# lucasjinreal/yolov7_d2

Hardware: AMD Instinct MI355X
Metric: images/sec training, YOLOX-s 640x640 bs=16/GPU (higher is better)
Workload: dtype bf16; 1 GPU; YOLOX-s CSPDarknet+PAFPN 640x640 bs=16/GPU: fwd + SimOTA loss + bwd + grad all-reduce + SGD(momentum) step, uint8 image batch + labels resident in HBM; global_batch=16, parallelism=dp1, hipgraph=True

## Files before the change

include/mi355_det.h:

```cpp
#ifndef MI355_DET_H
#define MI355_DET_H

#include <stdint.h>

#ifdef __cplusplus
extern "C" {
#endif

#define MI_OK 0
#define MI_EINVAL (-1)
#define MI_ELAUNCH (-2)
#define MI_ENODEV (-3)

typedef void* mi_stream_t;

int mi_version(void);
int mi_device_count(void);
const char* mi_last_error(void);

#define MI_CONV_ACCUM 1
#define MI_CONV_OUT_F32 2
#define MI_CONV_RELU 8
#define MI_CONV_RELUMASK 16
#define MI_CONV_ADDRELU 32
// ... 23 lines not shown
  int32_t KC, BN;
  int32_t stats_slots;
  int32_t TPS;
  const void* bn_y;
  const float* bn_scale;
  const float* bn_shift;
  const float* bn_mean;
  const float* bn_invstd;
  int32_t bn_ldy, bn_act;
  const void* xf;
  int32_t xf_write, xf_C;
} mi_conv_desc;

typedef struct mi_bnx {
  const void* res_unused; void* a;
  const float* gamma; const float* beta; float* rmean; float* rvar; int64_t* nbt;
  float* scale; float* shift; float* mean; float* invstd;
  int32_t ldres_unused, lda, act, pad0_;
  double inv_count, unbias;
  float eps, momentum;
  const double* acc;
  int32_t sld, nslots, C, pad1_;
} mi_bnx;

int mi_conv2d(const mi_conv_desc* d, mi_stream_t s);
int mi_conv2d_plan(mi_conv_desc* d);
int mi_conv2d_route(const mi_conv_desc* d);

#define MI_CONV_MAX_GROUP 8
typedef struct mi_conv_group {
  int32_t njobs, nblocks, lds_bytes;
  int32_t KC, BN, TPIX, TPS, EPI;
  int64_t starts_off, table_bytes;
  int64_t priv[288];
} mi_conv_group;
int mi_conv2d_group_plan(const mi_conv_desc* descs, int n, void* table_host, int64_t table_cap, mi_conv_group* meta);
int mi_conv2d_group_run(const mi_conv_group* meta, const void* table_dev, mi_stream_t s);

struct mi_bn_job;
int mi_conv2d_bn_plan(const mi_conv_desc* descs, const struct mi_bn_job* bn, int n, mi_conv_group* meta);
int mi_conv2d_bn_fwd(const mi_conv_desc* descs, const struct mi_bn_job* bn, int n, mi_stream_t s);
int mi_conv_bn_barrier_status(uint32_t* flags);

int mi_conv1x1_stream(const mi_conv_desc* descs, int n, mi_stream_t s);

int mi_conv3x3_ws(const mi_conv_desc* descs, int n, mi_stream_t s);

typedef struct mi_wgrad_desc {
  const void* x;
  const void* dy;
  float* gw;
  void* ws;
  int64_t ws_bytes;
  int32_t ldx, ldy;
  int32_t N, H, W, outH, outW;
  int32_t stride;
  int32_t Cin, Cout;
  int32_t CinPad, CoutPad;
  int32_t ntaps;
  int32_t tap_dy[MI_MAX_TAPS], tap_dx[MI_MAX_TAPS];
  int32_t accumulate;
  int32_t TH, TW, splitk, cfg_tp, cfg_ns;
  const float* row_scale;
  float* gbias;
} mi_wgrad_desc;
int mi_conv2d_wgrad(const mi_wgrad_desc* d, mi_stream_t s);
int64_t mi_conv2d_wgrad_plan(const mi_wgrad_desc* d);

#define MI_WGRAD_MAX_GROUPS 32
typedef struct mi_wgrad_group {
  int32_t ngroups, nred, red_blocks, pad_;
  struct {
    int32_t cfg[6];
    int32_t njobs, nblocks, lds_bytes, fixup;
    int64_t job_off, starts_off;
  } g[MI_WGRAD_MAX_GROUPS];
  int64_t red_off, red_starts_off, table_bytes, ws_bytes;
  int64_t red9_off, red9_starts_off;
  int32_t nred9, red9_blocks;
} mi_wgrad_group;
int mi_conv2d_wgrad_group_plan(const mi_wgrad_desc* descs, int n, void* ws_base, void* table_host,
                               int64_t table_cap, mi_wgrad_group* meta);
int mi_conv2d_wgrad_group_run(const mi_wgrad_group* meta, const void* table_dev, mi_stream_t s);
int mi_upload_async(void* dst_dev, const void* src_pinned, int64_t nbytes, mi_stream_t s);

int mi_pack_conv_weight(const float* w_oihw, int Cout, int Cin, int KH, int KW,
                        void* wf, int CinPad, int CoutPad,
                        void* wd, int CoutPadK, int CinPadN, mi_stream_t s);

int mi_pack_conv_weight_scaled(const float* w_oihw, const float* cout_scale, int Cout, int Cin, int KH, int KW,
                               void* wf, int CinPad, int CoutPad,
                               void* wd, int CoutPadK, int CinPadN, mi_stream_t s);
int mi_scale_rows_f32(const float* g, const float* scale, float* out, int rows, int rowlen, mi_stream_t s);

typedef struct mi_pack_job {
  const float* w;
  void* wf;
  void* wd;
  int32_t Cout, Cin, KK, CinPad, CoutPad, CoutPadK, CinPadN;
  int32_t blk0;
  const float* scale;
} mi_pack_job;
int mi_pack_jobs_layout(mi_pack_job* jobs_host, int njobs);
int mi_pack_conv_weights_batch(const mi_pack_job* jobs_dev, int njobs, int total_blocks, int kk_max, mi_stream_t s);

int mi_dwconv3x3_fwd(const void* x, int ldx, const float* w, void* y, int ldy, int N, int H, int W, int C, int stride,
                     int outH, int outW, double* stats_acc, int nslots, mi_stream_t s);
int mi_dwconv3x3_dgrad(const void* dy, int lddy, const float* w, void* dx, int lddx, int N, int H, int W, int C,
                       int stride, int outH, int outW, int accumulate, mi_stream_t s);
int64_t mi_dwconv3x3_wgrad_ws_bytes(int C);
int mi_dwconv3x3_wgrad(const void* x, int ldx, const void* dy, int lddy, int N, int H, int W, int C, int stride,
                       int outH, int outW, float* ws, int64_t ws_bytes, float* dw, mi_stream_t s);

#define MI_BN_MAX_GROUP 8
typedef struct mi_bn_job {
  const void* y; const void* res; void* a;
  const void* da; void* dy; void* dres;
  double* acc;
  const float* gamma; const float* beta; float* rmean; float* rvar; int64_t* nbt;
  float* scale; float* shift; float* mean; float* invstd; float* dgamma; float* dbeta;
  int64_t npix, count;
  int32_t ldy, ldres, lda, ldda, lddy, lddres, dres_accum, C, nslots, nblk, act, pad_;
  float eps, momentum;
  uint32_t* bar;
} mi_bn_job;
typedef struct mi_bn_group {
  int32_t kind, njobs, nblocks, act;
  int64_t starts_off, table_bytes;
} mi_bn_group;
int mi_bn_group_plan(int kind, const mi_bn_job* jobs, int n, void* table_host, int64_t table_cap, mi_bn_group* meta);
int mi_bn_group_run(const mi_bn_group* meta, const void* table_dev, mi_stream_t s);

int mi_bn_eval_affine(const float* gamma, const float* beta, const float* running_mean,
                      const float* running_var, float eps, int C, float* scale, float* shift,
                      mi_stream_t s);
int mi_bn_act_fwd(const void* y, int ldy, const double* stats_acc, int nslots, int64_t count, const float* gamma,
                  const float* beta, float eps, float momentum, float* running_mean, float* running_var,
                  int64_t* num_batches_tracked, float* scale, float* shift, float* mean, float* invstd,
                  const void* res, int ldres, void* a, int lda, int64_t npix, int C, int act, mi_stream_t s);
int mi_bn_act_bwd_reduce(const void* da, int ldda, const void* y, int ldy, const float* scale,
                         const float* shift, const float* mean, const float* invstd,
                         double* dacc, int nslots, int nblk, int64_t npix, int C, int act, mi_stream_t s);
int mi_bn_act_bwd_apply(const void* da, int ldda, const void* y, int ldy, const float* scale,
                        const float* shift, const float* mean, const float* invstd,
                        const float* gamma, const double* dacc, int nslots, int64_t count, float* dgamma,
                        float* dbeta,
                        void* dy, int lddy, void* dres, int lddres, int dres_accum, int64_t npix, int C, int act,
                        mi_stream_t s);
#define MI_BN_BAR_GROUPS 16
#define MI_BN_BAR_WORDS (64 * (1 + 2 * MI_BN_BAR_GROUPS))
int mi_bn_fused_set_capacity(int blocks);
int mi_bn_act_bwd_fused(const void* da, int ldda, const void* y, int ldy, const float* scale, const float* shift,
                        const float* mean, const float* invstd, const float* gamma, double* dacc, int nslots,
                        int64_t count, float* dgamma, float* dbeta, void* dy, int lddy, void* dres, int lddres,
                        int dres_accum, int64_t npix, int C, int act, uint32_t* barrier_words, mi_stream_t s);

int mi_focus_pack(const float* img_nchw, int N, int H, int W, void* out, int ldo, mi_stream_t s);
int mi_focus_pack_u8(const uint8_t* img_nchw, int N, int H, int W, void* out, int ldo, mi_stream_t s);
int mi_upsample2x_fwd(const void* x, int ldx, void* y, int ldy, int N, int H, int W, int C,
                      mi_stream_t s);
int mi_upsample2x_bwd(const void* dy, int lddy, void* dx, int lddx, int accumulate, int N, int H,
                      int W, int C, mi_stream_t s);
int mi_spp_pool_fwd(const void* x, int ldx, void* y5, void* y9, void* y13, int ldy, uint8_t* idx,
                    int N, int H, int W, int C, mi_stream_t s);
int mi_spp_pool_bwd(const void* dy5, const void* dy9, const void* dy13, int lddy,
                    const uint8_t* idx, void* dx, int lddx, int accumulate, int N, int H, int W,
// ... 161 lines not shown
} mi_mixup_job;
int mi_mixup_jobs_layout(mi_mixup_job* jobs_host, int njobs);
int mi_mixup_blend(const mi_mixup_job* jobs_dev, int njobs, int total_blocks, mi_stream_t s);

typedef struct mi_pil_resize_job {
  const void* src;
  void* tmp;
  void* dst;
  int64_t dsc, dsy, dsx;
  int64_t src_ld;
  double sat_src;
  int32_t h0, w0, nh, nw;
  int32_t hflip, vflip, shift_x, shift_y;
  int32_t src_hflip;
  int32_t color;
  float sat_dst, bri_dst;
  float dis_hue, dis_sat, dis_exp;
  int32_t dis_pos;
  int32_t blk0h, blk0v;
} mi_pil_resize_job;
int mi_pil_resize_jobs_layout(mi_pil_resize_job* jobs_host, int njobs, int32_t* blocks_h, int32_t* blocks_v);
int mi_pil_resize_h(const mi_pil_resize_job* jobs_dev, int njobs, int total_blocks, mi_stream_t s);
int mi_pil_resize_v(const mi_pil_resize_job* jobs_dev, int njobs, int total_blocks, mi_stream_t s);

typedef struct mi_jpeg_info {
  int32_t width, height, ncomp, restart_interval, orientation, adobe_transform;
  int32_t progressive, pad0_;
  int32_t comp_id[3], hs[3], vs[3], tq[3];
  int32_t hmax, vmax, mcu_w, mcu_h;
  int32_t blocks_w[3], blocks_h[3];
  int64_t coef_off[3], coef_count, sos_pos;
  uint16_t qt[4][64];
  uint8_t dc_bits[4][17], dc_vals[4][256], ac_bits[4][17], ac_vals[4][256];
  uint8_t have_qt[4], have_dc[4], have_ac[4], pad_[4];
} mi_jpeg_info;
typedef struct mi_jpeg_job {
  const int16_t* coef;
  void* planes;
  void* out;
  int64_t coef_off[3], plane_off[3];
  int32_t width, height, ncomp, orientation, bgr, ycc;
  int32_t hs[3], vs[3], blocks_w[3], blocks_h[3];
  int32_t hmax, vmax;
  int32_t blk0_idct, blk0_pix;
  uint16_t qt[3][64];
} mi_jpeg_job;
int mi_jpeg_parse(const uint8_t* data, int64_t len, mi_jpeg_info* info);
int mi_jpeg_huffman(const uint8_t* data, int64_t len, const mi_jpeg_info* info, int16_t* coef_host);
int mi_jpeg_huffman_batch(const uint8_t* const* datas, const int64_t* lens, const mi_jpeg_info* infos, int16_t* const* coefs_host,
                          int n, int threads, int32_t* rcs);
int mi_jpeg_job_fill(const mi_jpeg_info* info, const void* coef_dev, void* planes_dev, void* out_dev, int bgr,
                     int apply_orientation, mi_jpeg_job* job);
int mi_jpeg_jobs_layout(mi_jpeg_job* jobs_host, int njobs, int32_t* blocks_idct, int32_t* blocks_pix);
int mi_jpeg_idct(const mi_jpeg_job* jobs_dev, int njobs, int total_blocks, mi_stream_t s);
int mi_jpeg_color(const mi_jpeg_job* jobs_dev, int njobs, int total_blocks, mi_stream_t s);

int mi_rle_encode(const uint8_t* masks, int n, int H, int W, int max_runs, uint32_t* counts, int32_t* nruns, mi_stream_t s);
int mi_rle_to_string(const uint32_t* counts, int nruns, char* out, int out_cap);

int mi_batched_nms(const float* boxes, const float* scores, const float* idxs, int n, float iou_thr,
                   int32_t* order, uint64_t* mask, float* sboxes, int64_t* keep, int32_t* n_keep,
                   mi_stream_t s);
int mi_batched_nms_ex(const float* boxes, const float* scores, const float* idxs, int n, float iou_thr, int arithmetic,
                      int32_t* order, uint64_t* mask, float* sboxes, int64_t* keep, int32_t* n_keep, mi_stream_t s);
int64_t mi_yolox_postprocess_ws_bytes(int B, int A, int C);
int mi_yolox_postprocess(float* pred, int B, int A, int C, int ld, float conf_thr, float nms_thr, float* dets,
                         int32_t* counts, void* ws, int64_t ws_bytes, mi_stream_t s);
int mi_batched_softnms(const float* boxes, float* scores, const float* idxs, int n, float sigma, float score_threshold,
                       int linear, int64_t* keep, int32_t* n_keep, mi_stream_t s);
int mi_mask_nms(const float* inter, const float* sum_masks, const float* labels, int n, float nms_thr, uint8_t* keep,
                mi_stream_t s);
int mi_matrix_nms(const float* inter, const float* sum_masks, const float* labels, const float* scores, int n, float sigma,
                  int linear, float* comp_ws, float* out_scores, mi_stream_t s);

typedef struct mi_sgd_seg {
  int64_t offset, count;
  float weight_decay, lr;
} mi_sgd_seg;
int mi_sgd_momentum_step(float* params, const float* grads, float* momentum_buf,
                         const mi_sgd_seg* segs_dev, int nseg, float momentum, float grad_scale,
                         int first_step, mi_stream_t s);

int mi_sigmoid_f32(const float* x, const float* dy, float* y, float* dx, int64_t n, mi_stream_t s);
int mi_adamw_step(float* params, const float* grads, float* exp_avg, float* exp_avg_sq, const mi_sgd_seg* segs_dev,
                  int nseg, float beta1, float beta2, float eps, int64_t step, float grad_scale, mi_stream_t s);
typedef struct mi_adamw_tensor {
  float* p; const float* g; float* m; float* v;
  int64_t count;
  float lr, weight_decay;
} mi_adamw_tensor;
typedef struct mi_adamw_chunk {
  int32_t tensor, count;
  int64_t offset;
} mi_adamw_chunk;
int mi_adamw_step_multi(const mi_adamw_tensor* tensors_dev, const mi_adamw_chunk* chunks_dev, int nchunks, float beta1,
                        float beta2, float eps, const int64_t* step_dev, float grad_scale, mi_stream_t s);
int mi_grad_norm_multi(const mi_adamw_tensor* tensors_dev, const mi_adamw_chunk* chunks_dev, int nchunks,
                       double* partial_dev, float max_norm, float grad_scale, float* coef_norm_out, mi_stream_t s);
int mi_grad_gather_multi(const mi_adamw_tensor* tensors_dev, const mi_adamw_chunk* chunks_dev, int nchunks,
                         const int64_t* flat_off_dev, float* flat, mi_stream_t s);
int mi_adamw_step_multi_clip(const mi_adamw_tensor* tensors_dev, const mi_adamw_chunk* chunks_dev, int nchunks, float beta1,
                             float beta2, float eps, const int64_t* step_dev, float grad_scale,
                             const float* grad_scale_dev, mi_stream_t s);
int mi_grad_clip_full_model(float* grads, int64_t n, float max_norm, double* ws, float* norm_out, mi_stream_t s);
int mi_pos_embed_sine(const uint8_t* mask, int B, int H, int W, int num_pos_feats, float temperature, int normalize,
                      float scale, int centered, float* out, mi_stream_t s);

int mi_bilinear_resize_bf16(const void* x, int ldx, int N, int H, int W, int C, void* y, int ldy, int Ho, int Wo,
                            mi_stream_t s);
int mi_bilinear_resize_bwd_bf16(const void* dy, int lddy, int N, int H, int W, int C, void* dx, int lddx, int Ho, int Wo,
                                float* acc_ws_zeroed, mi_stream_t s);
#define MI_PYR_MAX_STAGES 8
int mi_pyramid_pool_fwd(const void* x, int ldx, int N, int H, int W, int C, int ns, const int* kh, const int* kw, void* const* y,
                        mi_stream_t s);
int mi_pyramid_pool_bwd(void* const* dy, int N, int H, int W, int C, int ns, const int* kh, const int* kw, void* dx, int lddx,
                        mi_stream_t s);
int64_t mi_sparseinst_mask_stats_ws_floats(int K, int P);
int mi_sparseinst_mask_stats(const void* masks, int ldm, int P, const float* targets, const int32_t* pairs, int K,
                             float* stats, float* ws, mi_stream_t s);
int mi_sparseinst_mask_grad(const void* masks, int ldm, int P, const float* targets, const int32_t* pairs, int K,
                            const float* stats, float c_bce, float c_dice, void* dmasks_zeroed, mi_stream_t s);
int mi_sparseinst_mask_grad_dev(const void* masks, int ldm, int P, const float* targets, const int32_t* pairs, int K,
                                const float* stats, const float* coef_dev, void* dmasks, mi_stream_t s);

typedef struct mi_sparseinst_loss_desc {
  const float* logits;
  const float* scores;
  const int64_t* labels;
  const int64_t* match_q;
  const int64_t* match_t;
  const int32_t* nmatch;
  const float* inv_num;
  const float* stats;
  const float* gup;
  int32_t* pairs;
  float* valid;
  int32_t* row_cls;
  int32_t* row_pair;
  float* kdev;
  float* losses;
  float* dlogits;
  float* dscores;
  float* coef;
  int B, N, C, cap, P, use_labels, use_masks, pad_;
  float alpha, gamma, w_ce, w_mask, w_dice, w_obj;
} mi_sparseinst_loss_desc;
int mi_sparseinst_match_cost(const float* num, const float* s2, const float* t2, const float* logits, const int64_t* labels,
                             int B, int N, int Np, int C, int cap, float alpha, float beta, float* cost, mi_stream_t s);
int mi_sparseinst_pairs(const mi_sparseinst_loss_desc* d, mi_stream_t s);
int mi_sparseinst_head_loss(const mi_sparseinst_loss_desc* d, mi_stream_t s);
int mi_sparseinst_head_loss_bwd(const mi_sparseinst_loss_desc* d, mi_stream_t s);

int mi_box_convert(const float* in, float* out, int64_t n, int to_cxcywh, mi_stream_t s);
int mi_box_iou_pairwise(const float* boxes1, int n, const float* boxes2, int m, float* iou, float* uni, float* giou,
                        int32_t* degenerate, mi_stream_t s);

int mi_abi_sizeof(int which);

typedef struct mi_cmd {
  int32_t op;
  int32_t i[40];
  float f[8];
  void* p[16];
  int64_t l[4];
} mi_cmd;

enum {
  MI_OP_NOP = 0,
  MI_OP_CONV = 1,
  MI_OP_WGRAD = 2,
  MI_OP_PACK_W = 3,
  MI_OP_RESERVED4 = 4,
  MI_OP_RESERVED5 = 5,
  MI_OP_BN_ACT_FWD = 6,
  MI_OP_BN_BWD_REDUCE = 7,
  MI_OP_RESERVED8 = 8,
  MI_OP_BN_BWD_APPLY = 9,
  MI_OP_FOCUS = 10,
  MI_OP_UPSAMPLE_FWD = 11,
  MI_OP_UPSAMPLE_BWD = 12,
  MI_OP_SPP_FWD = 13,
  MI_OP_SPP_BWD = 14,
  MI_OP_COPY = 15,
  MI_OP_COLSUM = 16,
  MI_OP_LOSS_FWD = 17,
  MI_OP_LOSS_BWD = 18,
  MI_OP_SPLIT_DPREDS = 19,
  MI_OP_MEMSET = 20,
  MI_OP_SGD = 21,
  MI_OP_BN_EVAL_AFFINE = 22,
  MI_OP_DECODE = 23,
  MI_OP_PACK_W_BATCH = 24,
  MI_OP_WGRAD_GROUP = 25,
  MI_OP_RESERVED26 = 26,
  MI_OP_RESERVED27 = 27,
  MI_OP_RESERVED28 = 28,
  MI_OP_BIAS_GRADS = 29,
  MI_OP_CONV_GROUP = 30,
  MI_OP_BN_GROUP = 31,
  MI_OP_SPLIT_DPREDS_BATCH = 32,
  MI_OP_BN_BWD_FUSED = 33,
  MI_OP_DWCONV_FWD = 34,
  MI_OP_DWCONV_DGRAD = 35,
  MI_OP_DWCONV_WGRAD = 36,
  MI_OP_LOSS_BWD_FUSED = 37,
  MI_OP_COUNT
};

int mi_cmdlist_run(const mi_cmd* cmds, int n, mi_stream_t s);
int64_t mi_graph_capture(const mi_cmd* cmds, int n, mi_stream_t s);
int mi_graph_launch(int64_t handle, mi_stream_t s);
int mi_graph_destroy(int64_t handle);

int mi_cmdlist_time(const mi_cmd* cmds, int n, int iters, float* ms, float* per_cmd_ms, mi_stream_t s);

#define MI_FEED_MAX_IMAGES 32
#define MI_FEED_MAX_LEVELS 8
typedef struct mi_image_job {
  const void* src;
  int h, w, dtype, pad_;
} mi_image_job;
typedef struct mi_mask_job {
  const void* masks;
  const int64_t* labels;
  int M, h, w, dtype;
} mi_mask_job;
int mi_normalize_pad_batch(const mi_image_job* jobs, int B, float* dst, int Hp, int Wp, const float* mean3, const float* std3,
                           mi_stream_t s);
int mi_padding_masks(const int64_t* sizes_dev, int B, int nlev, void* const* out, const int* H, const int* W, const int* stride,
                     mi_stream_t s);
int mi_mask_targets_batch(const mi_mask_job* jobs, int B, int cap, int Hi, int Wi, int Ho, int Wo, float* tgt, void* tgtT_bf16,
                          int64_t* labels, float* t2, float* t2_ws, mi_stream_t s);

#define MI_POLY_MAX_H 3807
typedef struct mi_poly_job {
  const double* verts;
  const int32_t* ring_off;
  const int32_t* inst_off;
  const int32_t* ring_off_host;
  const int32_t* inst_off_host;
  void* out;
  int M, h, w, pad_;
} mi_poly_job;
int mi_polygon_masks(const mi_poly_job* jobs, int B, mi_stream_t s);

typedef struct mi_sparseinst_infer_desc {
  int64_t out_off;
  int32_t n, h_img, w_img, Hout, Wout, pad_;
} mi_sparseinst_infer_desc;
int64_t mi_sparseinst_infer_ws_bytes(int B, int N, int h, int w);
int mi_sparseinst_infer_select(const float* logits, const float* obj, const void* masks, int mask_dtype, int64_t sb, int64_t sq,
                               int64_t sy, int64_t sx, int B, int N, int C, int h, int w, float cls_thr, float mask_thr,
                               int* counts, int* kept_query, float* scores, int64_t* labels, void* ws, int64_t ws_bytes,
                               mi_stream_t s);
int mi_sparseinst_infer_masks(const void* masks, int mask_dtype, int64_t sb, int64_t sq, int64_t sy, int64_t sx, int B, int N,
                              int h, int w, int Hpad, int Wpad, const int* kept_query, const mi_sparseinst_infer_desc* descs,
                              float mask_thr, void* out, int64_t out_bytes, mi_stream_t s);

int mi_probe_mfma32(const void* a_bf16_32x16, const void* b_bf16_16x32, float* d_32x32, mi_stream_t s);
int mi_probe_mfma16(const void* a_bf16_16x32, const void* b_bf16_32x16, float* d_16x16, mi_stream_t s);

#ifdef __cplusplus
}
#endif
#endif
```

yolov7_d2_amd/_lib.py:

```python
import ctypes as C
import os

_HERE = os.path.dirname(os.path.abspath(__file__))
LIB_PATH = os.environ.get("MI355_LIB", os.path.join(_HERE, "libmi355det.so"))

MI_MAX_TAPS = 16
MI_CONV_ACCUM = 1
MI_CONV_RELU = 8
MI_CONV_RELUMASK = 16
MI_CONV_ADDRELU = 32
MI_CONV_BNBWD = 4
MI_CONV_OUT_F32 = 2
MI_BN_BAR_WORDS = 64 * (1 + 2 * 16)
MI_BN_SLOTS = 16


class MI355Error(RuntimeError):
    pass


class mi_conv_desc(C.Structure):
    _fields_ = [
        ("x", C.c_void_p), ("w", C.c_void_p), ("y", C.c_void_p), ("bias", C.c_void_p),
        ("stats_acc", C.c_void_p),
# ... 44 lines not shown
                ("lr", C.c_float), ("weight_decay", C.c_float)]


class mi_adamw_chunk(C.Structure):
    _fields_ = [("tensor", C.c_int32), ("count", C.c_int32), ("offset", C.c_int64)]


class mi_bn_job(C.Structure):
    _fields_ = [(n, C.c_void_p) for n in ("y", "res", "a", "da", "dy", "dres", "acc", "gamma", "beta", "rmean", "rvar",
                                          "nbt", "scale", "shift", "mean", "invstd", "dgamma", "dbeta")] + \
               [("npix", C.c_int64), ("count", C.c_int64)] + \
               [(n, C.c_int32) for n in ("ldy", "ldres", "lda", "ldda", "lddy", "lddres", "dres_accum", "C", "nslots",
                                         "nblk", "act", "pad_")] + [("eps", C.c_float), ("momentum", C.c_float), ("bar", C.c_void_p)]


class mi_bn_group(C.Structure):
    _fields_ = [("kind", C.c_int32), ("njobs", C.c_int32), ("nblocks", C.c_int32), ("act", C.c_int32),
                ("starts_off", C.c_int64), ("table_bytes", C.c_int64)]


class mi_wgrad_desc(C.Structure):
    _fields_ = [
        ("x", C.c_void_p), ("dy", C.c_void_p), ("gw", C.c_void_p), ("ws", C.c_void_p), ("ws_bytes", C.c_int64),
        ("ldx", C.c_int32), ("ldy", C.c_int32),
        ("N", C.c_int32), ("H", C.c_int32), ("W", C.c_int32), ("outH", C.c_int32), ("outW", C.c_int32),
        ("stride", C.c_int32), ("Cin", C.c_int32), ("Cout", C.c_int32), ("CinPad", C.c_int32), ("CoutPad", C.c_int32),
        ("ntaps", C.c_int32),
        ("tap_dy", C.c_int32 * MI_MAX_TAPS), ("tap_dx", C.c_int32 * MI_MAX_TAPS),
        ("accumulate", C.c_int32),
        ("TH", C.c_int32), ("TW", C.c_int32), ("splitk", C.c_int32), ("cfg_tp", C.c_int32), ("cfg_ns", C.c_int32),
        ("row_scale", C.c_void_p), ("gbias", C.c_void_p),
    ]


class mi_yolox_loss_desc(C.Structure):
    _fields_ = [
        ("preds", C.c_void_p), ("labels", C.c_void_p), ("anchors", C.c_void_p),
        ("B", C.c_int32), ("A", C.c_int32), ("ncls", C.c_int32), ("max_labels", C.c_int32),
        ("gmax", C.c_int32),
        ("cost", C.c_void_p), ("iou", C.c_void_p), ("match", C.c_void_p), ("ngt", C.c_void_p),
        ("fg", C.c_void_p), ("matched_gt", C.c_void_p), ("matched_iou", C.c_void_p),
        ("partial", C.c_void_p), ("out", C.c_void_p), ("use_l1", C.c_int32), ("rsv_", C.c_int32), ("partial_l1", C.c_void_p),
        ("center_radius", C.c_float), ("cls_weight", C.c_float), ("iou_weight", C.c_float), ("reg_weight", C.c_float),
        ("iou_type", C.c_int32), ("rsv2_", C.c_int32),
    ]


class mi_sgd_seg(C.Structure):
    _fields_ = [("offset", C.c_int64), ("count", C.c_int64), ("weight_decay", C.c_float), ("lr", C.c_float)]


MI_WGRAD_MAX_GROUPS = 32


class _mi_wgrad_group_g(C.Structure):
    _fields_ = [("cfg", C.c_int32 * 6), ("njobs", C.c_int32), ("nblocks", C.c_int32), ("lds_bytes", C.c_int32),
                ("fixup", C.c_int32), ("job_off", C.c_int64), ("starts_off", C.c_int64)]


class mi_wgrad_group(C.Structure):
    _fields_ = [("ngroups", C.c_int32), ("nred", C.c_int32), ("red_blocks", C.c_int32), ("pad_", C.c_int32),
                ("g", _mi_wgrad_group_g * MI_WGRAD_MAX_GROUPS),
                ("red_off", C.c_int64), ("red_starts_off", C.c_int64), ("table_bytes", C.c_int64),
                ("ws_bytes", C.c_int64), ("red9_off", C.c_int64), ("red9_starts_off", C.c_int64),
                ("nred9", C.c_int32), ("red9_blocks", C.c_int32)]


class mi_bias_job(C.Structure):
    _fields_ = [("out", C.c_void_p), ("a0", C.c_int32), ("HW", C.c_int32), ("c0", C.c_int32), ("nc", C.c_int32)]


class mi_split_job(C.Structure):
    _fields_ = [("dst", C.c_void_p), ("a0", C.c_int32), ("HW", C.c_int32), ("c0", C.c_int32), ("nc", C.c_int32),
                ("ld", C.c_int32), ("rsv_", C.c_int32)]


class mi_pack_job(C.Structure):
    _fields_ = [("w", C.c_void_p), ("wf", C.c_void_p), ("wd", C.c_void_p),
                ("Cout", C.c_int32), ("Cin", C.c_int32), ("KK", C.c_int32), ("CinPad", C.c_int32),
                ("CoutPad", C.c_int32), ("CoutPadK", C.c_int32), ("CinPadN", C.c_int32), ("blk0", C.c_int32),
                ("scale", C.c_void_p)]


class mi_sparseinst_loss_desc(C.Structure):
    _fields_ = [(n, C.c_void_p) for n in ("logits", "scores", "labels", "match_q", "match_t", "nmatch", "inv_num", "stats", "gup",
                                          "pairs", "valid", "row_cls", "row_pair", "kdev", "losses", "dlogits", "dscores", "coef")] + \
               [(n, C.c_int32) for n in ("B", "N", "C", "cap", "P", "use_labels", "use_masks", "pad_")] + \
               [(n, C.c_float) for n in ("alpha", "gamma", "w_ce", "w_mask", "w_dice", "w_obj")]


class mi_image_job(C.Structure):
    _fields_ = [("src", C.c_void_p), ("h", C.c_int32), ("w", C.c_int32), ("dtype", C.c_int32), ("pad_", C.c_int32)]


class mi_mask_job(C.Structure):
    _fields_ = [("masks", C.c_void_p), ("labels", C.c_void_p), ("M", C.c_int32), ("h", C.c_int32), ("w", C.c_int32), ("dtype", C.c_int32)]


class mi_poly_job(C.Structure):
    _fields_ = [("verts", C.c_void_p), ("ring_off", C.c_void_p), ("inst_off", C.c_void_p), ("ring_off_host", C.c_void_p),
                ("inst_off_host", C.c_void_p), ("out", C.c_void_p), ("M", C.c_int32), ("h", C.c_int32), ("w", C.c_int32), ("pad_", C.c_int32)]


class mi_sparseinst_infer_desc(C.Structure):
    _fields_ = [("out_off", C.c_int64)] + [(n, C.c_int32) for n in ("n", "h_img", "w_img", "Hout", "Wout", "pad_")]


class mi_mosaic_paste_job(C.Structure):
    _fields_ = [("src", C.c_void_p), ("canvas", C.c_void_p)] + [(n, C.c_int32) for n in
                ("h0", "w0", "rh", "rw", "cw", "x1a", "y1a", "x2a", "y2a", "x1b", "y1b", "blk0", "fsrc", "pad_")]


class mi_warp_job(C.Structure):
    _fields_ = [("canvas", C.c_void_p), ("out", C.c_void_p), ("minv", C.c_double * 6)] + [(n, C.c_int32) for n in
                ("ch", "cw", "h", "w", "Hp", "Wp", "border", "blk0")]


class mi_mixup_job(C.Structure):
    _fields_ = [("src", C.c_void_p), ("out", C.c_void_p)] + [(n, C.c_int32) for n in
                ("h0", "w0", "rh1", "rw1", "dh", "dw", "oh", "ow", "flip", "x_off", "y_off", "th", "tw", "Hp", "Wp", "blk0", "fsrc", "pad_")]


class mi_pil_resize_job(C.Structure):
    _fields_ = ([("src", C.c_void_p), ("tmp", C.c_void_p), ("dst", C.c_void_p), ("dsc", C.c_int64), ("dsy", C.c_int64),
                 ("dsx", C.c_int64), ("src_ld", C.c_int64), ("sat_src", C.c_double)] +
                [(n, C.c_int32) for n in ("h0", "w0", "nh", "nw", "hflip", "vflip", "shift_x", "shift_y", "src_hflip", "color")] +
                [("sat_dst", C.c_float), ("bri_dst", C.c_float), ("dis_hue", C.c_float), ("dis_sat", C.c_float), ("dis_exp", C.c_float),
                 ("dis_pos", C.c_int32), ("blk0h", C.c_int32), ("blk0v", C.c_int32)])


class mi_jpeg_info(C.Structure):
    _fields_ = ([(n, C.c_int32) for n in ("width", "height", "ncomp", "restart_interval", "orientation", "adobe_transform",
                                         "progressive", "pad0_")] +
                [(n, C.c_int32 * 3) for n in ("comp_id", "hs", "vs", "tq")] +
                [(n, C.c_int32) for n in ("hmax", "vmax", "mcu_w", "mcu_h")] +
                [("blocks_w", C.c_int32 * 3), ("blocks_h", C.c_int32 * 3), ("coef_off", C.c_int64 * 3), ("coef_count", C.c_int64),
                 ("sos_pos", C.c_int64), ("qt", (C.c_uint16 * 64) * 4), ("dc_bits", (C.c_uint8 * 17) * 4),
                 ("dc_vals", (C.c_uint8 * 256) * 4), ("ac_bits", (C.c_uint8 * 17) * 4), ("ac_vals", (C.c_uint8 * 256) * 4),
                 ("have_qt", C.c_uint8 * 4), ("have_dc", C.c_uint8 * 4), ("have_ac", C.c_uint8 * 4), ("pad_", C.c_uint8 * 4)])


class mi_jpeg_job(C.Structure):
    _fields_ = ([("coef", C.c_void_p), ("planes", C.c_void_p), ("out", C.c_void_p), ("coef_off", C.c_int64 * 3),
                 ("plane_off", C.c_int64 * 3)] +
                [(n, C.c_int32) for n in ("width", "height", "ncomp", "orientation", "bgr", "ycc")] +
                [(n, C.c_int32 * 3) for n in ("hs", "vs", "blocks_w", "blocks_h")] +
                [(n, C.c_int32) for n in ("hmax", "vmax", "blk0_idct", "blk0_pix")] + [("qt", (C.c_uint16 * 64) * 3)])


class mi_cmd(C.Structure):
    _fields_ = [("op", C.c_int32), ("i", C.c_int32 * 40), ("f", C.c_float * 8), ("p", C.c_void_p * 16),
                ("l", C.c_int64 * 4)]


OPS = ["NOP", "CONV", "WGRAD", "PACK_W", "RESERVED4", "RESERVED5", "BN_ACT_FWD", "BN_BWD_REDUCE",
       "RESERVED8", "BN_BWD_APPLY", "FOCUS", "UPSAMPLE_FWD", "UPSAMPLE_BWD", "SPP_FWD", "SPP_BWD", "COPY",
       "COLSUM", "LOSS_FWD", "LOSS_BWD", "SPLIT_DPREDS", "MEMSET", "SGD", "BN_EVAL_AFFINE", "DECODE", "PACK_W_BATCH", "WGRAD_GROUP", "RESERVED26", "RESERVED27", "RESERVED28", "BIAS_GRADS",
       "CONV_GROUP", "BN_GROUP", "SPLIT_DPREDS_BATCH", "BN_BWD_FUSED", "DWCONV_FWD", "DWCONV_DGRAD", "DWCONV_WGRAD",
       "LOSS_BWD_FUSED"]
OP = {n: k for k, n in enumerate(OPS)}

_vp, _i, _i64, _f = C.c_void_p, C.c_int, C.c_int64, C.c_float
_PROTOS = {
    "mi_version": (C.c_int, []),
    "mi_device_count": (C.c_int, []),
    "mi_last_error": (C.c_char_p, []),
    "mi_conv2d": (C.c_int, [C.POINTER(mi_conv_desc), _vp]),
    "mi_conv2d_plan": (C.c_int, [C.POINTER(mi_conv_desc)]),
    "mi_conv2d_wgrad": (C.c_int, [C.POINTER(mi_wgrad_desc), _vp]),
    "mi_conv2d_wgrad_group_plan": (C.c_int, [C.POINTER(mi_wgrad_desc), _i, _vp, _vp, _i64, C.POINTER(mi_wgrad_group)]),
    "mi_conv2d_wgrad_group_run": (C.c_int, [C.POINTER(mi_wgrad_group), _vp, _vp]),
    "mi_pack_conv_weight": (C.c_int, [_vp, _i, _i, _i, _i, _vp, _i, _i, _vp, _i, _i, _vp]),
    "mi_pack_conv_weight_scaled": (C.c_int, [_vp, _vp, _i, _i, _i, _i, _vp, _i, _i, _vp, _i, _i, _vp]),
    "mi_scale_rows_f32": (C.c_int, [_vp, _vp, _vp, _i, _i, _vp]),
    "mi_conv2d_wgrad_plan": (C.c_int64, [C.POINTER(mi_wgrad_desc)]),
    "mi_bn_eval_affine": (C.c_int, [_vp, _vp, _vp, _vp, _f, _i, _vp, _vp, _vp]),
    "mi_bn_act_fwd": (C.c_int, [_vp, _i, _vp, _i, _i64, _vp, _vp, _f, _f, _vp, _vp, _vp, _vp, _vp, _vp, _vp, _vp, _i, _vp, _i,
                                _i64, _i, _i, _vp]),
    "mi_bn_act_bwd_reduce": (C.c_int, [_vp, _i, _vp, _i, _vp, _vp, _vp, _vp, _vp, _i, _i, _i64, _i, _i, _vp]),
    "mi_bn_act_bwd_apply": (C.c_int, [_vp, _i, _vp, _i, _vp, _vp, _vp, _vp, _vp, _vp, _i, _i64, _vp, _vp, _vp, _i, _vp, _i, _i,
                                      _i64, _i, _i, _vp]),
    "mi_focus_pack": (C.c_int, [_vp, _i, _i, _i, _vp, _i, _vp]),
    "mi_focus_pack_u8": (C.c_int, [_vp, _i, _i, _i, _vp, _i, _vp]),
    "mi_maxpool3x3s2_fwd": (C.c_int, [_vp, _i, _vp, _i, _i, _i, _i, _i, _vp]),
    "mi_maxpool3x3s2_bwd": (C.c_int, [_vp, _i, _vp, _i, _vp, _i, _i, _i, _i, _i, _i, _vp]),
    "mi_maxpool3x3s2_fwd_idx": (C.c_int, [_vp, _i, _vp, _i, _vp, _i, _i, _i, _i, _vp]),
    "mi_maxpool3x3s2_bwd_idx": (C.c_int, [_vp, _vp, _i, _vp, _i, _i, _i, _i, _i, _i, _vp]),
    "mi_upsample2x_fwd": (C.c_int, [_vp, _i, _vp, _i, _i, _i, _i, _i, _vp]),
    "mi_upsample2x_bwd": (C.c_int, [_vp, _i, _vp, _i, _i, _i, _i, _i, _i, _vp]),
    "mi_spp_pool_fwd": (C.c_int, [_vp, _i, _vp, _vp, _vp, _i, _vp, _i, _i, _i, _i, _vp]),
    "mi_spp_pool_bwd": (C.c_int, [_vp, _vp, _vp, _i, _vp, _vp, _i, _i, _i, _i, _i, _i, _vp]),
    "mi_copy_bf16": (C.c_int, [_vp, _i, _vp, _i, _i, _i64, _i, _vp]),
    "mi_colsum_bf16": (C.c_int, [_vp, _i, _i64, _i, _vp, _i, _vp, _vp]),
    "mi_colsum_bf16_wide": (C.c_int, [_vp, _i, _i64, _i, _vp, _i, _vp, _vp]),
    "mi_colsumsq_bf16_wide": (C.c_int, [_vp, _i, _i64, _i, _vp, _i, _vp, _vp]),
    "mi_colsum_wide_ws_bytes": (C.c_int64, [_i]),
    "mi_pack_conv_weights_batch": (C.c_int, [_vp, _i, _i, _i, _vp]),
    "mi_pack_jobs_layout": (C.c_int, [C.POINTER(mi_pack_job), _i]),
    "mi_yolox_loss_fwd": (C.c_int, [C.POINTER(mi_yolox_loss_desc), _vp]),
    "mi_yolox_loss_bwd": (C.c_int, [C.POINTER(mi_yolox_loss_desc), _vp, _vp, _vp]),
    "mi_yolox_loss_bwd_fused": (C.c_int, [C.POINTER(mi_yolox_loss_desc), _vp, _vp, C.POINTER(mi_split_job), _i,
                                          C.POINTER(mi_bias_job), _i, _vp, _i64, _vp]),
    "mi_yolox_split_dpreds": (C.c_int, [_vp, _i, _i, _i, _i, _i, _i, _i, _vp, _i, _vp]),
    "mi_yolox_split_dpreds_batch": (C.c_int, [_vp, _i, _i, _i, C.POINTER(mi_split_job), _i, _vp]),
    "mi_yolox_bias_grads": (C.c_int, [_vp, _i, _i, _i, C.POINTER(mi_bias_job), _i, _vp, _vp]),
    "mi_yolox_decode": (C.c_int, [_vp, _vp, _i, _i, _i, _vp]),
    "mi_hungarian_match": (C.c_int, [_vp, _vp, _vp, _vp, _vp, _i, _i, _i, _i, _f, _f, _f, _vp, _vp, _vp, _vp, _vp]),
    "mi_lsap": (C.c_int, [_vp, _vp, _i, _i, _i, _vp, _vp, _vp, _vp]),
    "mi_conv2d_group_plan": (C.c_int, [C.POINTER(mi_conv_desc), _i, _vp, _i64, C.POINTER(mi_conv_group)]),
    "mi_conv2d_group_run": (C.c_int, [C.POINTER(mi_conv_group), _vp, _vp]),
    "mi_conv2d_route": (C.c_int, [C.POINTER(mi_conv_desc)]),
    "mi_dropout_seed_offset": (C.c_int, [_vp]),
    "mi_adamw_step_multi": (C.c_int, [_vp, _vp, _i, _f, _f, _f, _vp, _f, _vp]),
    "mi_adamw_step_multi_clip": (C.c_int, [_vp, _vp, _i, _f, _f, _f, _vp, _f, _vp, _vp]),
    "mi_grad_norm_multi": (C.c_int, [_vp, _vp, _i, _vp, _f, _f, _vp, _vp]),
    "mi_grad_gather_multi": (C.c_int, [_vp, _vp, _i, _vp, _vp, _vp]),
    "mi_conv2d_bn_plan": (C.c_int, [C.POINTER(mi_conv_desc), C.POINTER(mi_bn_job), _i, C.POINTER(mi_conv_group)]),
    "mi_conv2d_bn_fwd": (C.c_int, [C.POINTER(mi_conv_desc), C.POINTER(mi_bn_job), _i, _vp]),
    "mi_conv_bn_barrier_status": (C.c_int, [C.POINTER(C.c_uint32)]),
    "mi_conv1x1_stream": (C.c_int, [C.POINTER(mi_conv_desc), _i, _vp]),
    "mi_conv3x3_ws": (C.c_int, [C.POINTER(mi_conv_desc), _i, _vp]),
    "mi_bn_act_bwd_fused": (C.c_int, [_vp, _i, _vp, _i, _vp, _vp, _vp, _vp, _vp, _vp, _i, _i64, _vp, _vp, _vp, _i, _vp, _i,
                                      _i, _i64, _i, _i, _vp, _vp]),
    "mi_bn_fused_set_capacity": (C.c_int, [_i]),
    "mi_dwconv3x3_fwd": (C.c_int, [_vp, _i, _vp, _vp, _i, _i, _i, _i, _i, _i, _i, _i, _vp, _i, _vp]),
    "mi_dwconv3x3_dgrad": (C.c_int, [_vp, _i, _vp, _vp, _i, _i, _i, _i, _i, _i, _i, _i, _i, _vp]),
    "mi_dwconv3x3_wgrad_ws_bytes": (C.c_int64, [_i]),
    "mi_dwconv3x3_wgrad": (C.c_int, [_vp, _i, _vp, _i, _i, _i, _i, _i, _i, _i, _i, _vp, _i64, _vp, _vp]),
    "mi_batched_nms_ex": (C.c_int, [_vp, _vp, _vp, _i, _f, _i, _vp, _vp, _vp, _vp, _vp, _vp]),
    "mi_batched_softnms": (C.c_int, [_vp, _vp, _vp, _i, _f, _f, _i, _vp, _vp, _vp]),
    "mi_mask_nms": (C.c_int, [_vp, _vp, _vp, _i, _f, _vp, _vp]),
    "mi_matrix_nms": (C.c_int, [_vp, _vp, _vp, _vp, _i, _f, _i, _vp, _vp, _vp]),
    "mi_groupnorm_ws_bytes": (C.c_int64, [_i, _i]),
    "mi_groupnorm_fwd": (C.c_int, [_vp, _i, _i, _i, _i, _i, _vp, _vp, _f, _vp, _i, _vp, _vp, _vp]),
    "mi_groupnorm_bwd": (C.c_int, [_vp, _i, _vp, _i, _i, _i, _i, _i, _vp, _vp, _vp, _i, _vp, _vp, _vp, _vp]),
    "mi_maxpool2x2_fwd": (C.c_int, [_vp, _i, _vp, _i, _i, _i, _i, _i, _vp]),
    "mi_maxpool2x2_bwd": (C.c_int, [_vp, _i, _vp, _i, _vp, _i, _i, _i, _i, _i, _vp]),
    "mi_fastattn_ws_bytes": (C.c_int64, []),
    "mi_fastattn_fwd": (C.c_int, [C.POINTER(C.c_void_p), _i, _vp, _vp, _i64, _vp]),
    "mi_fastattn_bwd": (C.c_int, [C.POINTER(C.c_void_p), _i, _vp, _vp, C.POINTER(C.c_void_p), _vp, _vp, _i64, _vp]),
    "mi_mosaic_jobs_layout": (C.c_int, [C.POINTER(mi_mosaic_paste_job), _i, C.POINTER(mi_warp_job), _i]),
    "mi_mosaic_paste": (C.c_int, [_vp, _i, _i, _vp]),
    "mi_warp_affine_u8": (C.c_int, [_vp, _i, _i, _vp]),
    "mi_mixup_jobs_layout": (C.c_int, [C.POINTER(mi_mixup_job), _i]),
    "mi_mixup_blend": (C.c_int, [_vp, _i, _i, _vp]),
    "mi_pil_resize_jobs_layout": (C.c_int, [C.POINTER(mi_pil_resize_job), _i, C.POINTER(C.c_int32), C.POINTER(C.c_int32)]),
    "mi_pil_resize_h": (C.c_int, [_vp, _i, _i, _vp]),
    "mi_pil_resize_v": (C.c_int, [_vp, _i, _i, _vp]),
    "mi_jpeg_parse": (C.c_int, [_vp, C.c_int64, C.POINTER(mi_jpeg_info)]),
    "mi_jpeg_huffman": (C.c_int, [_vp, C.c_int64, C.POINTER(mi_jpeg_info), _vp]),
    "mi_jpeg_huffman_batch": (C.c_int, [_vp, _vp, _vp, _vp, _i, _i, _vp]),
    "mi_jpeg_job_fill": (C.c_int, [C.POINTER(mi_jpeg_info), _vp, _vp, _vp, _i, _i, C.POINTER(mi_jpeg_job)]),
    "mi_jpeg_jobs_layout": (C.c_int, [C.POINTER(mi_jpeg_job), _i, C.POINTER(C.c_int32), C.POINTER(C.c_int32)]),
    "mi_jpeg_idct": (C.c_int, [_vp, _i, _i, _vp]),
# ... 130 lines not shown
```

yolov7_d2_amd/csrc/conv_wgrad.hip:

```cpp
#include <stdlib.h>
#include <string.h>
#include <vector>
#include "common.h"

struct Wg2K {
  const __bf16* x;
  const __bf16* dy;
  float* part;
  int ldx, lddy, N, H, W, outH, outW, is;
  int TH, TW, tilesY, tilesX, ntiles, tps, nsplit;
  int dymin, dxmin, haloW, npixh, nqx, stage, ns;
  int toff[MI_MAX_TAPS];
  int nco, nci;
  int nrx;
  int xmap;
  unsigned mTW, mHW;
  long long V;
  float* bpart;
  int bld, fix;
  float* g;
  const float* row_scale;
  int Cout, Cin, accumulate, pad_;
  int ra, rb;
  long long cnt_rel;
};

__device__ uint4 g_mi_zero_page[4];

typedef __attribute__((address_space(3))) s16x4* lds_s16x4_ptr;

__device__ __forceinline__ bf16x8 tr_read2(const char* base0, const char* base1) {
  const s16x4 lo = __builtin_amdgcn_ds_read_tr16_b64_v4i16((lds_s16x4_ptr)(base0));
  const s16x4 hi = __builtin_amdgcn_ds_read_tr16_b64_v4i16((lds_s16x4_ptr)(base1));
  typedef __attribute__((ext_vector_type(8))) short s16x8;
  s16x8 v;
  v[0] = lo[0]; v[1] = lo[1]; v[2] = lo[2]; v[3] = lo[3];
  v[4] = hi[0]; v[5] = hi[1]; v[6] = hi[2]; v[7] = hi[3];
  return __builtin_bit_cast(bf16x8, v);
}

__device__ __forceinline__ void glds16(const void* g, unsigned lds_off) {
  asm volatile("s_mov_b32 m0, %1\n\ts_nop 0\n\tglobal_load_lds_dwordx4 %0, off" ::"v"(g), "s"(__builtin_amdgcn_readfirstlane(lds_off)) : "memory", "m0");
}

__device__ __forceinline__ void wait_vmcnt(int n) {
#define MI_VMC(k) case k: asm volatile("s_waitcnt vmcnt(" #k ")" ::: "memory"); break;
  switch (n < 0 ? 0 : (n > 30 ? 30 : n)) {
    MI_VMC(0) MI_VMC(1) MI_VMC(2) MI_VMC(3) MI_VMC(4) MI_VMC(5) MI_VMC(6) MI_VMC(7) MI_VMC(8) MI_VMC(9) MI_VMC(10)
    MI_VMC(11) MI_VMC(12) MI_VMC(13) MI_VMC(14) MI_VMC(15) MI_VMC(16) MI_VMC(17) MI_VMC(18) MI_VMC(19) MI_VMC(20)
    MI_VMC(21) MI_VMC(22) MI_VMC(23) MI_VMC(24) MI_VMC(25) MI_VMC(26) MI_VMC(27) MI_VMC(28) MI_VMC(29) MI_VMC(30)
  }
#undef MI_VMC
}

template <int NG>
__device__ __forceinline__ int swz32(int row) {
  if (NG == 1) return 0;
  if (NG == 2) return (row >> 2) & 1;
  if (NG == 4) return (row >> 1) & 3;
  return row & 7;
}

template <int NTHR, int BCO>
struct WgBias {
  static constexpr int NCH = BCO / 8, RL = NTHR / NCH;
  float s[8];
  __device__ __forceinline__ void init() {
#pragma unroll
    for (int e = 0; e < 8; ++e) s[e] = 0.f;
  }
  template <int TP>
  __device__ __forceinline__ void tile(const Wg2K& p, const int img, const int ty0, const int tx0, const int co0, const int TPv) {
    const int tid = threadIdx.x, ch = tid % NCH, rl = tid / NCH;
    if (rl >= RL) return;
    const __bf16* const dyb = p.dy + ((size_t)img * p.outH * p.outW) * (size_t)p.lddy + co0 + ch * 8;
    constexpr int NR = (TP + RL - 1) / RL;
    bf16x8 v[NR];
#pragma unroll
    for (int k = 0; k < NR; ++k) {
      const int row = rl + k * RL;
      const int ty = (int)(((unsigned)row * p.mTW) >> 20);
      const int tx = row - ty * p.TW;
      const int oy = ty0 + ty, ox = tx0 + tx;
      const bool ok = (row < TPv) & (oy < p.outH) & (ox < p.outW);
#pragma unroll
      for (int e = 0; e < 8; ++e) v[k][e] = (__bf16)0.f;
// ... 519 lines not shown
#pragma unroll
    for (int ks = 0; ks < KS; ++ks) {
      bf16x8 a[MI];
#pragma unroll
      for (int i = 0; i < MI; ++i)
        a[i] = tr_read2(aB + (i * TP + ks * 32) * 32, aB + (i * TP + ks * 32 + 16) * 32);
      const char* const b0 = sB + hb[ks][0];
      const char* const b1 = sB + hb[ks][1];
#pragma unroll
      for (int tap = 0; tap < NT; ++tap) {
        bf16x8 b[NJ];
#pragma unroll
        for (int j = 0; j < NJ; ++j)
          b[j] = tr_read2(b0 + toff32[tap] + j * jstride, b1 + toff32[tap] + j * jstride);
#pragma unroll
        for (int i = 0; i < MI; ++i)
#pragma unroll
          for (int j = 0; j < NJ; ++j)
            acc[tap][i][j] = __builtin_amdgcn_mfma_f32_16x16x32_bf16(a[i], b[j], acc[tap][i][j], 0, 0, 0);
      }
    }
  }
  f32x4* out = (f32x4*)p.part + (size_t)s * (size_t)p.V +
               ((size_t)((cob * p.nci + cib) * NW + wave) * (NT * MI * NJ)) * 64 + lane;
  if (FIX) {
    const __amdgpu_buffer_rsrc_t rs = wg_slab_rsrc(p.part);
    const unsigned ob = (unsigned)(((size_t)s * (size_t)p.V + ((size_t)((cob * p.nci + cib) * NW + wave) * (NT * MI * NJ)) * 64 + lane) * 16);
#pragma unroll
    for (int tap = 0; tap < NT; ++tap)
#pragma unroll
      for (int i = 0; i < MI; ++i)
#pragma unroll
        for (int j = 0; j < NJ; ++j) st_agent16(rs, ob, (unsigned)(((tap * MI + i) * NJ + j) * 1024), acc[tap][i][j]);
    wg_fixup<NT, MI, NJ, WCO, WCI>(p, cnt, s, cob * p.nci + cib, smem);
    return;
  }
#pragma unroll
  for (int tap = 0; tap < NT; ++tap)
#pragma unroll
    for (int i = 0; i < MI; ++i)
#pragma unroll
      for (int j = 0; j < NJ; ++j) out[((tap * MI + i) * NJ + j) * 64] = acc[tap][i][j];
  if (p.bpart != nullptr) {
    if (do_bias) bias.finish(p, (float*)smem, s, co0);
  }
}

template <int NT, int MI, int NJ, int WCO, int WCI, int TP>
__global__ __launch_bounds__(WCO* WCI * 64, 2) void wgrad3_kernel(const Wg2K p) {
  wgrad3_body<NT, MI, NJ, WCO, WCI, TP>(p, blockIdx.x);
}
template <int NT, int MI, int NJ, int WCO, int WCI, int TP>
__global__ __launch_bounds__(WCO* WCI * 64, 2) void wgrad3_group_kernel(const Wg2K* __restrict__ jobs,
                                                                         const int* __restrict__ starts, int njobs) {
  const int b = blockIdx.x;
  int j = 0;
  while (j + 1 < njobs && starts[j + 1] <= b) ++j;
  const Wg2K p = jobs[j];
  wgrad3_body<NT, MI, NJ, WCO, WCI, TP>(p, b - starts[j]);
}
template <int TP>
__global__ __launch_bounds__(256, 2) void wgrad3_multi_kernel(const Wg2K* __restrict__ jobs, const int* __restrict__ starts, int njobs) {
  const int b = blockIdx.x;
  int j = 0;
  while (j + 1 < njobs && starts[j + 1] <= b) ++j;
  const Wg2K p = jobs[j];
  const int bid = b - starts[j];
  switch (p.pad_) {
    case 0x41: wgrad3_body<9, 4, 1, 1, 4, TP>(p, bid); break;
    case 0x22: wgrad3_body<9, 2, 1, 2, 2, TP>(p, bid); break;
    default: wgrad3_body<9, 1, 1, 2, 2, TP>(p, bid); break;
  }
}
template <int NT, int MI, int NJ, int WCO, int WCI, int TP>
__global__ __launch_bounds__(WCO* WCI * 64, 2) void wgrad3_group_fix_kernel(const Wg2K* __restrict__ jobs,
                                                                             const int* __restrict__ starts, int njobs) {
  const int b = blockIdx.x;
  int j = 0;
  while (j + 1 < njobs && starts[j + 1] <= b) ++j;
  const Wg2K p = jobs[j];
  wgrad3_body<NT, MI, NJ, WCO, WCI, TP, true>(p, b - starts[j], (unsigned*)((char*)const_cast<Wg2K*>(jobs) + p.cnt_rel));
}

struct Wg2R {
  const f32x4* part;
  float* g;
  long long V;
  int nsplit, NT, MI, NJ, WCO, WCI, nco, nci, Cout, Cin, accumulate;
  const float* row_scale;
  const float* bpart;
  float* gbias;
  int bld, main_blocks;
};
__device__ __forceinline__ void wgrad2_reduce_bias(const Wg2R& p, const long long blk) {
  const int c = (int)(blk - p.main_blocks) * 256 + (int)threadIdx.x;
  if (c >= p.Cout) return;
  float a = 0.f;
  for (int k = 0; k < p.nsplit; ++k) a += p.bpart[(size_t)k * p.bld + c];
  p.gbias[c] = a;
}

template <int SL>
__device__ __forceinline__ void wgrad2_reduce_body(const Wg2R& p, const long long blk) {
  constexpr int OUTS = 256 / SL;
  __shared__ f32x4 red[SL > 1 ? SL - 1 : 1][OUTS];
  const int o = threadIdx.x % OUTS, sl = threadIdx.x / OUTS;
  const long long v = blk * OUTS + o;
  const bool valid = v < p.V;
  f32x4 s0 = {0.f, 0.f, 0.f, 0.f}, s1 = s0, s2 = s0, s3 = s0;
  if (valid) {
    const f32x4* src = p.part + v;
    int k = sl;
    for (; k + 3 * SL < p.nsplit; k += 4 * SL) {
      const f32x4 a = src[(size_t)k * p.V], b = src[(size_t)(k + SL) * p.V], c = src[(size_t)(k + 2 * SL) * p.V],
                  d = src[(size_t)(k + 3 * SL) * p.V];
      s0 += a; s1 += b; s2 += c; s3 += d;
    }
    for (; k < p.nsplit; k += SL) s0 += src[(size_t)k * p.V];
  }
  f32x4 sum = (s0 + s1) + (s2 + s3);
  if (SL > 1) {
    if (sl > 0) red[sl - 1][o] = sum;
    __syncthreads();
    if (sl > 0) return;
#pragma unroll
    for (int q = 0; q < SL - 1; ++q) sum += red[q][o];
  }
  if (!valid) return;
  wg_scatter(p.g, p.row_scale, p.accumulate, p.NT, p.MI, p.NJ, p.WCO, p.WCI, p.nci, p.Cout, p.Cin, v, sum);
}

__device__ __forceinline__ void wgrad2_reduce9_body(const Wg2R& p, const int blk) {
  __shared__ float tile[16 * 16 * 9 + 16];
  const int tid = threadIdx.x, lane = tid & 63, tap = tid >> 6;
  int r = blk;
  const int j = r % p.NJ; r /= p.NJ;
  const int i = r % p.MI; r /= p.MI;
  const int NW = p.WCO * p.WCI;
  const int wave = r % NW; r /= NW;
  const int cib = r % p.nci, cob = r / p.nci;
  const long long v = ((((long long)(r * NW + wave) * 9 + tap) * p.MI + i) * p.NJ + j) * 64 + lane;
  f32x4 s0 = {0.f, 0.f, 0.f, 0.f}, s1 = s0, s2 = s0, s3 = s0;
  const f32x4* src = p.part + v;
  int k = 0;
  for (; k + 4 <= p.nsplit; k += 4) {
    const f32x4 a = src[(size_t)k * p.V], b = src[(size_t)(k + 1) * p.V], c = src[(size_t)(k + 2) * p.V],
                d = src[(size_t)(k + 3) * p.V];
    s0 += a; s1 += b; s2 += c; s3 += d;
  }
  for (; k < p.nsplit; ++k) s0 += src[(size_t)k * p.V];
  const f32x4 sum = (s0 + s1) + (s2 + s3);
#pragma unroll
  for (int e = 0; e < 4; ++e) tile[((4 * (lane >> 4) + e) * 16 + (lane & 15)) * 9 + tap] = sum[e];
  __syncthreads();
  const int wco = wave / p.WCI, wci = wave % p.WCI;
  const int ci0 = cib * (16 * p.NJ * p.WCI) + (wci * p.NJ + j) * 16;
  const int co0 = cob * (16 * p.MI * p.WCO) + (wco * p.MI + i) * 16;
  if (ci0 >= p.Cin) return;
  const int row = tid / 36, c4 = (tid % 36) * 4;
  const int co = co0 + row;
  const int nval = min(16, p.Cin - ci0) * 9;
  if (co >= p.Cout || c4 >= nval) return;
  float* dst = p.g + ((size_t)co * p.Cin + ci0) * 9 + c4;
  const float* t = tile + row * 144 + c4;
  const float rs = p.row_scale ? p.row_scale[co] : 1.f;
  if (c4 + 4 <= nval && ((uintptr_t)dst & 15) == 0) {
    f32x4 o = {t[0] * rs, t[1] * rs, t[2] * rs, t[3] * rs};
    if (p.accumulate) o += *(const f32x4*)dst;
    *(f32x4*)dst = o;
  } else {
    for (int e = 0; e < 4 && c4 + e < nval; ++e) dst[e] = p.accumulate ? dst[e] + t[e] * rs : t[e] * rs;
  }
}
__global__ __launch_bounds__(576) void wgrad2_reduce9_kernel(const Wg2R p) { wgrad2_reduce9_body(p, blockIdx.x); }
__global__ __launch_bounds__(576) void wgrad2_reduce9_group_kernel(const Wg2R* __restrict__ jobs,
                                                                   const int* __restrict__ starts, int njobs) {
// ... 442 lines not shown
        done[j] = 1;
        starts.push_back(blocks);
        ks[j].pad_ = cs[j].NT == 9 ? cs[j].MI * 16 + cs[j].WCO : cs[j].MI * 16 + cs[j].NJ;
        if (fix) {
          ks[j].fix = 1;
          ks[j].cnt_rel = (long long)cnt_off[j] - (long long)job_off;
        }
        jobs.push_back(ks[j]);
        blocks += ks[j].nsplit * ks[j].nco * ks[j].nci;
        if (ldss[j] > lds) lds = ldss[j];
      }
    starts.push_back(blocks);
    if (fix) {
      const size_t need = 16 + (size_t)3 * WG_FIX_U * (cs[i].WCO * cs[i].WCI * 16) * 16;
      if (lds < need) lds = need;
    }
    g.njobs = (int)jobs.size(); g.nblocks = blocks; g.lds_bytes = (int32_t)lds; g.fixup = fix ? 1 : 0;
    g.job_off = put(jobs.data(), jobs.size() * sizeof(Wg2K));
    MI_REQUIRE(g.job_off == job_off, "wgrad_group_plan: table layout");
    g.starts_off = put(starts.data(), starts.size() * sizeof(int));
  }
  std::vector<Wg2R> rj, rj9;
  std::vector<int> rs, rs9;
  int rblocks = 0, rblocks9 = 0;
  for (int i = 0; i < n && !fix; ++i) {
    Wg2R r;
    r.part = (const f32x4*)ks[i].part; r.g = descs[i].gw; r.V = ks[i].V; r.nsplit = ks[i].nsplit;
    r.NT = cs[i].NT; r.MI = cs[i].MI; r.NJ = cs[i].NJ; r.WCO = cs[i].WCO; r.WCI = cs[i].WCI;
    r.nco = ks[i].nco; r.nci = ks[i].nci; r.Cout = descs[i].Cout; r.Cin = descs[i].Cin;
    r.accumulate = descs[i].accumulate; r.row_scale = descs[i].row_scale;
    r.bpart = nullptr; r.gbias = nullptr; r.bld = 0; r.main_blocks = 0;
    if (descs[i].gbias) {
      const int outs = 256 / wg_redsl();
      r.bpart = ks[i].bpart; r.gbias = descs[i].gbias; r.bld = ks[i].bld;
      r.main_blocks = (int)((ks[i].V + outs - 1) / outs);
      rj.push_back(r);
      rs.push_back(rblocks);
      rblocks += r.main_blocks + (descs[i].Cout + 255) / 256;
      continue;
    }
    if (cs[i].NT == 9 && wg_red9()) {
      rj9.push_back(r);
      rs9.push_back(rblocks9);
      rblocks9 += (int)(ks[i].V / (64 * 9));
    } else {
      rj.push_back(r);
      rs.push_back(rblocks);
      const int outs = 256 / wg_redsl();
      rblocks += (int)((ks[i].V + outs - 1) / outs);
    }
  }
  rs.push_back(rblocks);
  rs9.push_back(rblocks9);
  meta->nred = (int)rj.size(); meta->red_blocks = rblocks;
  meta->red_off = put(rj.data(), rj.size() * sizeof(Wg2R));
  meta->red_starts_off = put(rs.data(), rs.size() * sizeof(int));
  meta->nred9 = (int)rj9.size(); meta->red9_blocks = rblocks9;
  meta->red9_off = put(rj9.data(), rj9.size() * sizeof(Wg2R));
  meta->red9_starts_off = put(rs9.data(), rs9.size() * sizeof(int));
  meta->table_bytes = (int64_t)off;
  if (tab) MI_REQUIRE((int64_t)off <= table_cap, "wgrad_group_plan: table needs %zu bytes", off);
  return MI_OK;
}

template <int NT, int MI, int NJ, int WCO, int WCI, int TP>
static int wg_group_launch(const Wg2K* jobs, const int* starts, int njobs, int nblocks, size_t lds, hipStream_t s, bool fix) {
  auto fn = fix ? (wg_use_v3(NT) ? wgrad3_group_fix_kernel<NT, MI, NJ, WCO, WCI, TP> : wgrad2_group_fix_kernel<NT, MI, NJ, WCO, WCI, TP>)
                : (wg_use_v3(NT) ? wgrad3_group_kernel<NT, MI, NJ, WCO, WCI, TP> : wgrad2_group_kernel<NT, MI, NJ, WCO, WCI, TP>);
  static bool attr_done = false;
  if (!attr_done) {
    hipFuncSetAttribute((const void*)wgrad2_group_kernel<NT, MI, NJ, WCO, WCI, TP>, hipFuncAttributeMaxDynamicSharedMemorySize, 160 * 1024);
    hipFuncSetAttribute((const void*)wgrad3_group_kernel<NT, MI, NJ, WCO, WCI, TP>, hipFuncAttributeMaxDynamicSharedMemorySize, 160 * 1024);
    hipFuncSetAttribute((const void*)wgrad2_group_fix_kernel<NT, MI, NJ, WCO, WCI, TP>, hipFuncAttributeMaxDynamicSharedMemorySize, 160 * 1024);
    hipFuncSetAttribute((const void*)wgrad3_group_fix_kernel<NT, MI, NJ, WCO, WCI, TP>, hipFuncAttributeMaxDynamicSharedMemorySize, 160 * 1024);
    attr_done = true;
  }
  if ((size_t)wg_min_lds() > lds && wg_min_lds() <= 160 * 1024) lds = (size_t)wg_min_lds();
  hipLaunchKernelGGL(fn, dim3((unsigned)nblocks), dim3(WCO * WCI * 64), lds, s, jobs, starts, njobs);
  MI_CHECK_LAUNCH("conv_wgrad_group");
  return MI_OK;
}

extern "C" int mi_conv2d_wgrad_group_run(const mi_wgrad_group* meta, const void* table_dev, mi_stream_t st) {
  MI_REQUIRE(meta && table_dev && meta->ngroups > 0, "wgrad_group_run: args");
  hipStream_t s = (hipStream_t)st;
  const char* tab = (const char*)table_dev;
  for (int gi = 0; gi < meta->ngroups; ++gi) {
    const auto& g = meta->g[gi];
    const Wg2K* jobs = (const Wg2K*)(tab + g.job_off);
    const int* starts = (const int*)(tab + g.starts_off);
    int rc = MI_EINVAL;
#define MI_WG(NTv, MIv, NJv, WCOv, WCIv, TPv)                                                                   \
  if (g.cfg[0] == NTv && g.cfg[1] == MIv && g.cfg[2] == NJv && g.cfg[3] == WCOv && g.cfg[4] == WCIv &&          \
      g.cfg[5] == TPv)                                                                                          \
    rc = wg_group_launch<NTv, MIv, NJv, WCOv, WCIv, TPv>(jobs, starts, g.njobs, g.nblocks, (size_t)g.lds_bytes, s, g.fixup == 1);
    MI_WG_ALL
#undef MI_WG
    if (g.cfg[0] == 1 && g.cfg[1] == 0 && g.cfg[2] == 0 && g.fixup != 1) {
      static bool attr_done = false;
      if (!attr_done) {
        hipFuncSetAttribute((const void*)wgrad2_multi_kernel<64>, hipFuncAttributeMaxDynamicSharedMemorySize, 160 * 1024);
        hipFuncSetAttribute((const void*)wgrad2_multi_kernel<128>, hipFuncAttributeMaxDynamicSharedMemorySize, 160 * 1024);
        attr_done = true;
      }
      if (g.cfg[5] == 64)
        hipLaunchKernelGGL(wgrad2_multi_kernel<64>, dim3((unsigned)g.nblocks), dim3(256), (size_t)g.lds_bytes, s, jobs, starts, g.njobs);
      else
        hipLaunchKernelGGL(wgrad2_multi_kernel<128>, dim3((unsigned)g.nblocks), dim3(256), (size_t)g.lds_bytes, s, jobs, starts, g.njobs);
      MI_CHECK_LAUNCH("conv_wgrad_multi");
      rc = MI_OK;
    }
    if (g.cfg[0] == 9 && g.cfg[1] == 0 && g.cfg[2] == 0 && g.fixup != 1) {
      static bool attr_done = false;
      if (!attr_done) {
        hipFuncSetAttribute((const void*)wgrad3_multi_kernel<64>, hipFuncAttributeMaxDynamicSharedMemorySize, 160 * 1024);
        hipFuncSetAttribute((const void*)wgrad3_multi_kernel<128>, hipFuncAttributeMaxDynamicSharedMemorySize, 160 * 1024);
        attr_done = true;
      }
      if (g.cfg[5] == 64)
        hipLaunchKernelGGL(wgrad3_multi_kernel<64>, dim3((unsigned)g.nblocks), dim3(256), (size_t)g.lds_bytes, s, jobs, starts, g.njobs);
      else
        hipLaunchKernelGGL(wgrad3_multi_kernel<128>, dim3((unsigned)g.nblocks), dim3(256), (size_t)g.lds_bytes, s, jobs, starts, g.njobs);
      MI_CHECK_LAUNCH("conv_wgrad3_multi");
      rc = MI_OK;
    }
    if (rc == MI_EINVAL) MI_FAIL(MI_EINVAL, "wgrad_group: no kernel for group %d", gi);
    if (rc) return rc;
  }
  if (meta->red9_blocks > 0) {
    hipLaunchKernelGGL(wgrad2_reduce9_group_kernel, dim3((unsigned)meta->red9_blocks), dim3(576), 0, s,
                       (const Wg2R*)(tab + meta->red9_off), (const int*)(tab + meta->red9_starts_off), meta->nred9);
    MI_CHECK_LAUNCH("conv_wgrad_reduce9_group");
  }
  if (meta->red_blocks > 0) {
    const dim3 g((unsigned)meta->red_blocks);
    const Wg2R* jt = (const Wg2R*)(tab + meta->red_off);
    const int* st_ = (const int*)(tab + meta->red_starts_off);
    switch (wg_redsl()) {
      case 16: hipLaunchKernelGGL(wgrad2_reduce_group_kernel<16>, g, dim3(256), 0, s, jt, st_, meta->nred); break;
      case 8: hipLaunchKernelGGL(wgrad2_reduce_group_kernel<8>, g, dim3(256), 0, s, jt, st_, meta->nred); break;
      case 4: hipLaunchKernelGGL(wgrad2_reduce_group_kernel<4>, g, dim3(256), 0, s, jt, st_, meta->nred); break;
      default: hipLaunchKernelGGL(wgrad2_reduce_group_kernel<1>, g, dim3(256), 0, s, jt, st_, meta->nred);
    }
    MI_CHECK_LAUNCH("conv_wgrad_reduce_group");
  }
  return MI_OK;
}
```

yolov7_d2_amd/csrc/misc_ops.hip:

```cpp
#include <stdlib.h>
#include "common.h"

static int ew_blocks(int64_t total, int cap = 4096) {
  int64_t b = (total + 255) / 256;
  if (b > cap) b = cap;
  if (b < 1) b = 1;
  return (int)b;
}

__global__ __launch_bounds__(256) void focus_pack_kernel(const float* __restrict__ img, int N, int H, int W,
                                                         __bf16* out, int ldo) {
  const int Ho = H / 2, Wo = W / 2;
  const int64_t total = (int64_t)N * Ho * Wo;
  for (int64_t idx = blockIdx.x * 256LL + threadIdx.x; idx < total; idx += (int64_t)gridDim.x * 256) {
    const int ox = (int)(idx % Wo);
    const int64_t r = idx / Wo;
    const int oy = (int)(r % Ho), n = (int)(r / Ho);
    float f[16];
#pragma unroll
    for (int q = 0; q < 4; ++q) {
      const int dy = q & 1, dx = q >> 1;
#pragma unroll
      for (int c = 0; c < 3; ++c)
        f[q * 3 + c] = img[(((int64_t)n * 3 + c) * H + (2 * oy + dy)) * W + 2 * ox + dx];
    }
    f[12] = f[13] = f[14] = f[15] = 0.f;
    __bf16* op = out + idx * ldo;
    *(bf16x8*)op = pack8(f);
    *(bf16x8*)(op + 8) = pack8(f + 8);
  }
}

template <class T>
__global__ __launch_bounds__(256) void focus_pack4_kernel(const T* __restrict__ img, int N, int H, int W, __bf16* out,
                                                          int ldo) {
  const int Ho = H / 2, Wo = W / 2;
  const unsigned total = (unsigned)N * (unsigned)Ho * (unsigned)Wo;
  const unsigned stride = gridDim.x * 256u;
  for (unsigned idx0 = blockIdx.x * 256u + threadIdx.x; idx0 < total; idx0 += 4 * stride) {
    float f[4][16];
#pragma unroll
    for (int j = 0; j < 4; ++j) {
      const unsigned idx = idx0 + j * stride;
      if (idx >= total) break;
      const unsigned r = idx / (unsigned)Wo;
      const int ox = (int)(idx - r * (unsigned)Wo);
      const unsigned nn = r / (unsigned)Ho;
      const int oy = (int)(r - nn * (unsigned)Ho), n = (int)nn;
#pragma unroll
      for (int c = 0; c < 3; ++c)
#pragma unroll
        for (int dy = 0; dy < 2; ++dy) {
          const T* src = img + (((int64_t)n * 3 + c) * H + (2 * oy + dy)) * W + 2 * ox;
          if constexpr (sizeof(T) == 4) {
            const float2 v = *(const float2*)src;
            f[j][dy * 3 + c] = v.x;
            f[j][(2 + dy) * 3 + c] = v.y;
          } else {
            const unsigned short v = *(const unsigned short*)src;
            f[j][dy * 3 + c] = (float)(v & 0xff);
            f[j][(2 + dy) * 3 + c] = (float)(v >> 8);
          }
        }
      f[j][12] = f[j][13] = f[j][14] = f[j][15] = 0.f;
    }
#pragma unroll
    for (int j = 0; j < 4; ++j) {
      const unsigned idx = idx0 + j * stride;
      if (idx >= total) break;
      __bf16* op = out + (size_t)idx * ldo;
      *(bf16x8*)op = pack8(f[j]);
      *(bf16x8*)(op + 8) = pack8(f[j] + 8);
    }
  }
}

#define FOCUS_ROWS 2
__global__ __launch_bounds__(256) void focus_pack_u8_rows_kernel(const uint8_t* __restrict__ img, int N, int H, int W,
                                                                 __bf16* out, int ldo) {
  extern __shared__ __attribute__((aligned(16))) uint8_t srow[];
  const int Ho = H / 2, Wo = W / 2;
  const int rb = (Ho + FOCUS_ROWS - 1) / FOCUS_ROWS;
  const int n = blockIdx.x / rb, oy0 = (blockIdx.x % rb) * FOCUS_ROWS;
  const int per = W / 16;
// ... 700 lines not shown
    const int c = tid & 63, q = tid >> 6, nbk = (int)gridDim.x;
    float a = 0.f;
    if (c < C8N * 8) {
      int b = q;
      for (; b + 12 < nbk; b += 16) {
        float v[4];
#pragma unroll
        for (int u = 0; u < 4; ++u) v[u] = __hip_atomic_load(part + (size_t)(b + 4 * u) * CP + c0 + c, __ATOMIC_RELAXED, __HIP_MEMORY_SCOPE_AGENT);
        a += (v[0] + v[1]) + (v[2] + v[3]);
      }
      for (; b < nbk; b += 4) a += __hip_atomic_load(part + (size_t)b * CP + c0 + c, __ATOMIC_RELAXED, __HIP_MEMORY_SCOPE_AGENT);
    }
    red[q * 64 + c] = a;
    __syncthreads();
    if (tid < C8N * 8 && c0 + tid < C) {
      const float t = (red[tid] + red[64 + tid]) + (red[128 + tid] + red[192 + tid]);
      out[c0 + tid] = accumulate ? out[c0 + tid] + t : t;
    }
  }
}
extern "C" int64_t mi_colsum_wide_ws_bytes(int C) { return (int64_t)128 * ((C + 7) / 8 * 8) * 4; }
static int colsum_wide_launch(const void* x, int ldx, int64_t npix, int C, float* out, int accumulate, float* ws, int sq,
                              mi_stream_t st) {
  MI_REQUIRE(x && out && ws && C > 0, "colsum_wide: null / C %d", C);
  const int CP = (C + 7) / 8 * 8;
  MI_REQUIRE(ldx % 8 == 0 && ((uintptr_t)x % 16) == 0 && ldx >= CP, "colsum_wide: alignment / ld");
  hipStream_t s = (hipStream_t)st;
  int nblk = (int)((npix + 255) / 256);
  if (nblk > 128) nblk = 128;
  if (nblk < 1) nblk = 1;
  const char* two_e = getenv("MI_COLSUM_TWO_STAGE");
  const int two = two_e ? atoi(two_e) : 0;
  if ((CP + 63) / 64 <= COLSUM_MAX_CHUNKS && !two) {
    hipLaunchKernelGGL(colsum_wide_fused_kernel, dim3(nblk, (CP + 63) / 64), dim3(256), 0, s, (const __bf16*)x, ldx, npix, CP, C, ws,
                       out, accumulate, sq);
    MI_CHECK_LAUNCH("colsum_wide");
    return MI_OK;
  }
  hipLaunchKernelGGL(colsum_wide_stage1_kernel, dim3(nblk, (CP + 63) / 64), dim3(256), 0, s, (const __bf16*)x, ldx, npix, CP, ws, sq);
  MI_CHECK_LAUNCH("colsum_wide1");
  hipLaunchKernelGGL(colsum_wide_stage2_kernel, dim3((C + 127) / 128), dim3(128), 0, s, ws, nblk, CP, C, out, accumulate);
  MI_CHECK_LAUNCH("colsum_wide2");
  return MI_OK;
}
extern "C" int mi_colsum_bf16_wide(const void* x, int ldx, int64_t npix, int C, float* out, int accumulate, float* ws,
                                   mi_stream_t st) {
  return colsum_wide_launch(x, ldx, npix, C, out, accumulate, ws, 0, st);
}
extern "C" int mi_colsumsq_bf16_wide(const void* x, int ldx, int64_t npix, int C, float* out, int accumulate, float* ws,
                                     mi_stream_t st) {
  return colsum_wide_launch(x, ldx, npix, C, out, accumulate, ws, 1, st);
}

__global__ __launch_bounds__(256) void scale_rows_kernel(const float* __restrict__ g, const float* __restrict__ sc, float* out,
                                                         int rows, int rowlen) {
  const int64_t n = (int64_t)rows * rowlen;
  if ((rowlen & 3) == 0) {
    const int64_t n4 = n >> 2;
    const int rl4 = rowlen >> 2;
    for (int64_t i = blockIdx.x * 256LL + threadIdx.x; i < n4; i += (int64_t)gridDim.x * 256) {
      const float f = sc[i / rl4];
      float4 v = ((const float4*)g)[i];
      v.x *= f; v.y *= f; v.z *= f; v.w *= f;
      ((float4*)out)[i] = v;
    }
  } else {
    for (int64_t i = blockIdx.x * 256LL + threadIdx.x; i < n; i += (int64_t)gridDim.x * 256) out[i] = g[i] * sc[i / rowlen];
  }
}
extern "C" int mi_scale_rows_f32(const float* g, const float* scale, float* out, int rows, int rowlen, mi_stream_t st) {
  MI_REQUIRE(g && scale && out && rows > 0 && rowlen > 0, "scale_rows: args");
  MI_REQUIRE(((uintptr_t)g % 16) == 0 && ((uintptr_t)out % 16) == 0, "scale_rows: alignment");
  int64_t blocks = ((int64_t)rows * rowlen / 4 + 255) / 256;
  if (blocks > 2048) blocks = 2048;
  if (blocks < 1) blocks = 1;
  hipLaunchKernelGGL(scale_rows_kernel, dim3((int)blocks), dim3(256), 0, (hipStream_t)st, g, scale, out, rows, rowlen);
  MI_CHECK_LAUNCH("scale_rows");
  return MI_OK;
}

__global__ __launch_bounds__(256) void sgd_kernel(float* p, const float* __restrict__ g, float* m,
                                                  const mi_sgd_seg* __restrict__ segs, float momentum,
                                                  float grad_scale, int first_step) {
  const mi_sgd_seg sg = segs[blockIdx.x];
  const float wd = sg.weight_decay, lr = sg.lr;
  const int64_t n4 = ((sg.offset & 3) == 0) ? (sg.count >> 2) : 0;
  f32x4* p4 = (f32x4*)(p + sg.offset);
  const f32x4* g4 = (const f32x4*)(g + sg.offset);
  f32x4* m4 = (f32x4*)(m + sg.offset);
  for (int64_t i = threadIdx.x; i < n4; i += 512) {
    const bool two = i + 256 < n4;
    const f32x4 pa = p4[i], ga = g4[i], ma = first_step ? f32x4{0.f, 0.f, 0.f, 0.f} : m4[i];
    f32x4 pb = {0.f, 0.f, 0.f, 0.f}, gb = pb, mb = pb;
    if (two) {
      pb = p4[i + 256];
      gb = g4[i + 256];
      if (!first_step) mb = m4[i + 256];
    }
    f32x4 da = ga * grad_scale + pa * wd;
    f32x4 ba = first_step ? da : ma * momentum + da;
    m4[i] = ba;
    p4[i] = pa - ba * lr;
    if (two) {
      f32x4 db = gb * grad_scale + pb * wd;
      f32x4 bb = first_step ? db : mb * momentum + db;
      m4[i + 256] = bb;
      p4[i + 256] = pb - bb * lr;
    }
  }
  for (int64_t i = n4 * 4 + threadIdx.x; i < sg.count; i += 256) {
    const int64_t k = sg.offset + i;
    const float pv = p[k];
    const float d = g[k] * grad_scale + wd * pv;
    const float b = first_step ? d : momentum * m[k] + d;
    m[k] = b;
    p[k] = pv - lr * b;
  }
}
extern "C" int mi_sgd_momentum_step(float* params, const float* grads, float* momentum_buf,
                                    const mi_sgd_seg* segs_dev, int nseg, float momentum, float grad_scale,
                                    int first_step, mi_stream_t st) {
  MI_REQUIRE(params && grads && momentum_buf && segs_dev && nseg > 0, "sgd: args");
  hipLaunchKernelGGL(sgd_kernel, dim3(nseg), dim3(256), 0, (hipStream_t)st, params, grads, momentum_buf, segs_dev,
                     momentum, grad_scale, first_step);
  MI_CHECK_LAUNCH("sgd");
  return MI_OK;
}
```

yolov7_d2_amd/csrc/runtime.hip:

```cpp
#include <mutex>
#include <unordered_map>
#include <vector>
#include "common.h"

__global__ __launch_bounds__(256) void fill16_kernel(u32x4* p, size_t n16, unsigned v) {
  const u32x4 w = {v, v, v, v};
  for (size_t k = (size_t)blockIdx.x * 256 + threadIdx.x; k < n16; k += (size_t)gridDim.x * 256) p[k] = w;
}

thread_local char g_mi_err[512] = {0};

extern "C" int mi_version(void) { return 100; }
extern "C" const char* mi_last_error(void) { return g_mi_err; }

const unsigned long long* g_mi_seed_off = nullptr;
extern "C" int mi_dropout_seed_offset(const uint64_t* dev_word) {
  g_mi_seed_off = (const unsigned long long*)dev_word;
  return MI_OK;
}
extern "C" int mi_device_count(void) {
  int n = 0;
  if (hipGetDeviceCount(&n) != hipSuccess) return 0;
  return n;
}

static int run_one(const mi_cmd& c, hipStream_t s) {
  mi_stream_t st = (mi_stream_t)s;
  const int32_t* i = c.i;
  void* const* p = c.p;
  switch (c.op) {
    case MI_OP_NOP: return MI_OK;
    case MI_OP_CONV: return mi_conv2d((const mi_conv_desc*)p[0], st);
    case MI_OP_WGRAD: return mi_conv2d_wgrad((const mi_wgrad_desc*)p[0], st);
    case MI_OP_PACK_W:
      return mi_pack_conv_weight((const float*)p[0], i[0], i[1], i[2], i[3], p[1], i[4], i[5], p[2], i[6], i[7], st);
    case MI_OP_BN_ACT_FWD:
      return mi_bn_act_fwd(p[0], i[0], (const double*)p[1], i[5], c.l[0], (const float*)p[2], (const float*)p[3], c.f[0],
                           c.f[1], (float*)p[4], (float*)p[5], (int64_t*)p[6], (float*)p[7], (float*)p[8],
                           (float*)p[9], (float*)p[10], p[11], i[1], p[12], i[2], c.l[1], i[3], i[4], st);
    case MI_OP_BN_BWD_REDUCE:
      return mi_bn_act_bwd_reduce(p[0], i[0], p[1], i[1], (const float*)p[2], (const float*)p[3], (const float*)p[4],
                                  (const float*)p[5], (double*)p[6], i[5], i[2], c.l[0], i[3], i[4], st);
    case MI_OP_BN_BWD_APPLY:
      return mi_bn_act_bwd_apply(p[0], i[0], p[1], i[1], (const float*)p[2], (const float*)p[3], (const float*)p[4],
                                 (const float*)p[5], (const float*)p[6], (const double*)p[7], i[7], c.l[1], (float*)p[8],
                                 (float*)p[9], p[10], i[2], p[11], i[3], i[4], c.l[0], i[5], i[6], st);
    case MI_OP_BN_BWD_FUSED:
      return mi_bn_act_bwd_fused(p[0], i[0], p[1], i[1], (const float*)p[2], (const float*)p[3], (const float*)p[4],
                                 (const float*)p[5], (const float*)p[6], (double*)p[7], i[7], c.l[1], (float*)p[8],
                                 (float*)p[9], p[10], i[2], p[11], i[3], i[4], c.l[0], i[5], i[6], (uint32_t*)p[12], st);
    case MI_OP_DWCONV_FWD:
      return mi_dwconv3x3_fwd(p[0], i[0], (const float*)p[1], p[2], i[1], i[2], i[3], i[4], i[5], i[6], i[7], i[8],
                              (double*)p[3], i[9], st);
    case MI_OP_DWCONV_DGRAD:
      return mi_dwconv3x3_dgrad(p[0], i[0], (const float*)p[1], p[2], i[1], i[2], i[3], i[4], i[5], i[6], i[7], i[8], i[9], st);
    case MI_OP_DWCONV_WGRAD:
      return mi_dwconv3x3_wgrad(p[0], i[0], p[1], i[1], i[2], i[3], i[4], i[5], i[6], i[7], i[8], (float*)p[2], c.l[0],
                                (float*)p[3], st);
    case MI_OP_FOCUS:
      return i[4] ? mi_focus_pack_u8((const uint8_t*)p[0], i[0], i[1], i[2], p[1], i[3], st)
                  : mi_focus_pack((const float*)p[0], i[0], i[1], i[2], p[1], i[3], st);
    case MI_OP_UPSAMPLE_FWD: return mi_upsample2x_fwd(p[0], i[0], p[1], i[1], i[2], i[3], i[4], i[5], st);
    case MI_OP_UPSAMPLE_BWD: return mi_upsample2x_bwd(p[0], i[0], p[1], i[1], i[2], i[3], i[4], i[5], i[6], st);
    case MI_OP_SPP_FWD: return mi_spp_pool_fwd(p[0], i[0], p[1], p[2], p[3], i[1], (uint8_t*)p[4], i[2], i[3], i[4], i[5], st);
    case MI_OP_SPP_BWD:
      return mi_spp_pool_bwd(p[0], p[1], p[2], i[0], (const uint8_t*)p[3], p[4], i[1], i[2], i[3], i[4], i[5], i[6], st);
    case MI_OP_COPY: return mi_copy_bf16(p[0], i[0], p[1], i[1], i[2], c.l[0], i[3], st);
    case MI_OP_COLSUM: return mi_colsum_bf16(p[0], i[0], c.l[0], i[1], (float*)p[1], i[2], (float*)p[2], st);
    case MI_OP_BIAS_GRADS:
      return mi_yolox_bias_grads((const float*)p[1], i[0], i[1], i[2], (const mi_bias_job*)p[0], i[3], (float*)p[2], st);
    case MI_OP_WGRAD_GROUP: return mi_conv2d_wgrad_group_run((const mi_wgrad_group*)p[0], p[1], st);
    case MI_OP_CONV_GROUP: return mi_conv2d_group_run((const mi_conv_group*)p[0], p[1], st);
    case MI_OP_BN_GROUP: return mi_bn_group_run((const mi_bn_group*)p[0], p[1], st);
    case MI_OP_PACK_W_BATCH: return mi_pack_conv_weights_batch((const mi_pack_job*)p[0], i[0], i[1], i[2], st);
    case MI_OP_LOSS_FWD: return mi_yolox_loss_fwd((const mi_yolox_loss_desc*)p[0], st);
    case MI_OP_LOSS_BWD_FUSED:
      return mi_yolox_loss_bwd_fused((const mi_yolox_loss_desc*)p[0], (const float*)p[1], (float*)p[2], (const mi_split_job*)p[3], i[0],
                                     (const mi_bias_job*)p[4], i[1], (float*)p[5], c.l[0], st);
    case MI_OP_LOSS_BWD: return mi_yolox_loss_bwd((const mi_yolox_loss_desc*)p[0], (const float*)p[1], (float*)p[2], st);
    case MI_OP_SPLIT_DPREDS:
      return mi_yolox_split_dpreds((const float*)p[0], i[0], i[1], i[2], i[3], i[4], i[5], i[6], p[1], i[7], st);
    case MI_OP_SPLIT_DPREDS_BATCH:
      return mi_yolox_split_dpreds_batch((const float*)p[1], i[0], i[1], i[2], (const mi_split_job*)p[0], i[3], st);
    case MI_OP_MEMSET: {
      const size_t n = (size_t)c.l[0];
      if (((uintptr_t)p[0] % 16) == 0 && n % 16 == 0 && n > 0 && n < ((size_t)1 << 40)) {
        const unsigned v = (unsigned)(i[0] & 0xff) * 0x01010101u;
        const size_t n16 = n / 16;
        size_t nb = (n16 + 255) / 256;
        if (nb > 2048) nb = 2048;
        hipLaunchKernelGGL(fill16_kernel, dim3((unsigned)nb), dim3(256), 0, s, (u32x4*)p[0], n16, v);
        MI_CHECK_LAUNCH("memset (fill kernel)");
        return MI_OK;
      }
      if (hipMemsetAsync(p[0], i[0], n, s) != hipSuccess) MI_FAIL(MI_ELAUNCH, "memset failed");
      return MI_OK;
    }
    case MI_OP_SGD:
      return mi_sgd_momentum_step((float*)p[0], (const float*)p[1], (float*)p[2], (const mi_sgd_seg*)p[3], i[0],
                                  c.f[0], c.f[1], i[1], st);
    case MI_OP_BN_EVAL_AFFINE:
      return mi_bn_eval_affine((const float*)p[0], (const float*)p[1], (const float*)p[2], (const float*)p[3], c.f[0],
                               i[0], (float*)p[4], (float*)p[5], st);
    case MI_OP_DECODE: return mi_yolox_decode((float*)p[0], (const float*)p[1], i[0], i[1], i[2], st);
    default: MI_FAIL(MI_EINVAL, "cmdlist: unknown op %d", c.op);
  }
}

extern "C" int mi_cmdlist_run(const mi_cmd* cmds, int n, mi_stream_t st) {
  if (mi_device_count() <= 0) MI_FAIL(MI_ENODEV, "no HIP device");
  hipStream_t s = (hipStream_t)st;
  for (int k = 0; k < n; ++k) {
    const int rc = run_one(cmds[k], s);
    if (rc != MI_OK) {
      char tmp[400];
      snprintf(tmp, sizeof(tmp), "%s", g_mi_err);
      snprintf(g_mi_err, sizeof(g_mi_err), "cmd %d (op %d): %s", k, cmds[k].op, tmp);
      return rc;
    }
  }
  return MI_OK;
}

extern "C" int mi_upload_async(void* dst_dev, const void* src_pinned, int64_t nbytes, mi_stream_t st) {
  MI_REQUIRE(dst_dev && src_pinned && nbytes > 0, "upload_async: args");
  const hipError_t e = hipMemcpyAsync(dst_dev, src_pinned, (size_t)nbytes, hipMemcpyHostToDevice, (hipStream_t)st);
  if (e != hipSuccess) MI_FAIL(MI_ELAUNCH, "upload_async: %s", hipGetErrorString(e));
  return MI_OK;
}

static std::mutex g_graph_mu;
static std::unordered_map<int64_t, hipGraphExec_t> g_graphs;
static int64_t g_next_graph = 1;

extern "C" int64_t mi_graph_capture(const mi_cmd* cmds, int n, mi_stream_t st) {
  if (mi_device_count() <= 0) MI_FAIL(MI_ENODEV, "no HIP device");
  hipStream_t s = (hipStream_t)st;
  if (s == nullptr) MI_FAIL(MI_EINVAL, "graph capture needs a non-default stream");
  if (hipStreamBeginCapture(s, hipStreamCaptureModeThreadLocal) != hipSuccess)
    MI_FAIL(MI_ELAUNCH, "hipStreamBeginCapture failed");
  const int rc = mi_cmdlist_run(cmds, n, st);
  hipGraph_t graph = nullptr;
  const hipError_t e = hipStreamEndCapture(s, &graph);
  if (rc != MI_OK) {
    if (graph) (void)hipGraphDestroy(graph);
    return rc;
  }
  if (e != hipSuccess || !graph) MI_FAIL(MI_ELAUNCH, "hipStreamEndCapture: %s", hipGetErrorString(e));
  hipGraphExec_t exec = nullptr;
  const hipError_t e2 = hipGraphInstantiate(&exec, graph, nullptr, nullptr, 0);
  (void)hipGraphDestroy(graph);
  if (e2 != hipSuccess) MI_FAIL(MI_ELAUNCH, "hipGraphInstantiate: %s", hipGetErrorString(e2));
  std::lock_guard<std::mutex> lk(g_graph_mu);
  const int64_t h = g_next_graph++;
// ... 123 lines not shown
```

yolov7_d2_amd/engine.py:

```python
import ctypes as C
import os

import torch
import torch.distributed as dist
import torch.nn as nn

from . import _lib as L
from .parallel import GradReducer, broadcast_params, grad_write_ranges, plan_buckets


def ddp_schedule(plan, builder, params, world, n_buckets=3, group=None):
    writes = grad_write_ranges(plan, params.grad)
    bounds = None
    if world > 1 and getattr(builder, "wgrad_split", False):
        bounds = []
        for pre in builder.wgrad_stages:
            offs = [o for (name, p, o, n) in params.entries if name.startswith(tuple(pre))]
            if offs:
                bounds.append(min(offs))
    buckets = plan_buckets(params.total, writes, n_buckets if world > 1 else 1, bounds=bounds or None)
    red = GradReducer(params.grad, buckets, group=group)
    barr, bn = plan.bwd_cmds
    return red, red.segments(bn)


class NativeTrainer:
    def __init__(self, model, lr=0.01, momentum=0.9, weight_decay=1e-4, weight_decay_norm=0.0, n_buckets=3,
                 use_graph=True, loss_weights=(1.0, 1.0, 1.0, 1.0), tune=None, input_u8=False):
        self.model = model
        self.input_u8 = bool(input_u8)
        self.copy_stream = None
        self._feed = None
        self.feed_direct = os.environ.get("MI_FEED_DIRECT", "1") != "0"
        self.one_graph = os.environ.get("MI_STEP_ONE_GRAPH", "1") != "0"
        model.train()
        self.params = model.ensure_params()
        self.world = dist.get_world_size() if dist.is_initialized() else 1
        ov = os.environ.get("MI_DDP_OVERLAP", "auto")
        self.ddp_mode = None if self.world == 1 else {"1": "overlap", "0": "exposed"}.get(ov)
        self.ddp_auto = self.world > 1 and self.ddp_mode is None
        self.ddp_choice = None
        self._bn_capacity_full = L.lib().mi_bn_fused_set_capacity(0) if self.world > 1 else 0
        broadcast_params(self.params.data)
        norm_ids = set()
        for m in model.modules():
            if isinstance(m, nn.BatchNorm2d):
                norm_ids.update(id(p) for p in m.parameters())
        self.segs, self.nseg = self.params.build_sgd_segments(lr, weight_decay, weight_decay_norm, norm_ids)
        self.momentum, self.n_buckets, self.use_graph = momentum, n_buckets, use_graph
        self.loss_weights = loss_weights
        self._states = {}
        self.stream = torch.cuda.Stream()
        self.tune = (os.environ.get("MI_CONV_TUNE", "0") == "1") if tune is None else bool(tune)
        self.tune_report = None

    def set_lr(self, lr):
        with torch.cuda.stream(self.stream):
            self.params.set_lr(lr)

    def _ddp_build_env(self, mode):
        full = self._bn_capacity_full
        if mode == "exposed":
            L.lib().mi_bn_fused_set_capacity(0)
            return {"MI_WGRAD_SPLIT": "0", "MI_BN_FUSED": os.environ.get("MI_BN_FUSED", "auto")}
        L.lib().mi_bn_fused_set_capacity(full - full // 8)
        return {}

    def _state(self, B, H, W, mode=None):
        primary = self.ddp_mode or ("overlap" if self.world > 1 else None)
        mode = mode or primary
        key = (B, H, W) if mode == primary else (B, H, W, mode)
        st = self._states.get(key)
        if st is not None:
            return st
        env = self._ddp_build_env(mode) if self.world > 1 else {}
        prev = {k: os.environ.get(k) for k in env}
        os.environ.update(env)
        try:
            variant = "ddp-exposed" if mode == "exposed" else ""
            ps = self.model.plan_for(B, H, W, True, input_u8=self.input_u8, variant=variant)
        finally:
            for k, v in prev.items():
                if v is None:
                    os.environ.pop(k, None)
                else:
                    os.environ[k] = v
        ps.gw().copy_(torch.tensor(self.loss_weights, dtype=torch.float32))
        plan = ps.plan
        sgd = (L.mi_cmd * 1)()
        sgd[0].op = L.OP["SGD"]
        sgd[0].p[0], sgd[0].p[1], sgd[0].p[2], sgd[0].p[3] = (self.params.data.data_ptr(), self.params.grad.data_ptr(),
                                                             self.params.mom.data_ptr(), self.segs.data_ptr())
        sgd[0].i[0], sgd[0].i[1] = self.nseg, 0
        sgd[0].f[0], sgd[0].f[1] = self.momentum, 1.0 / self.world
        red, segs = ddp_schedule(plan, ps.builder, self.params, self.world, 1 if mode == "exposed" else self.n_buckets)
        st = dict(ps=ps, plan=plan, sgd=sgd, red=red, segs=segs, graphs=None, ddp_mode=mode)
        self._states[key] = st
        return st

    def _run_backward(self, st):
        lib, sp = L.lib(), L.stream_ptr(self.stream)
        barr, bn = st["plan"].bwd_cmds
        gs = st["graphs"] if self.use_graph else None
        for i, (lo, hi, bucket) in enumerate(st["segs"]):
            if gs:
                if gs["bwd"][i] is not None:
                    L.check(lib.mi_graph_launch(gs["bwd"][i], sp), "launch bwd")
            else:
                self._run_cmds(barr, lo, hi, sp)
            st["red"].reduce_bucket(bucket)
        st["red"].wait()

    def _choose_ddp_schedule(self, st, rounds=3, reps=3):
        lib, sp = L.lib(), L.stream_ptr(self.stream)
        B, H, W = st["ps"].B, st["ps"].H, st["ps"].W
        saved = [(t, t.clone()) for t in getattr(st["ps"].builder, "tune_restore", [])]
        with torch.cuda.stream(self.stream):
            st2 = self._state(B, H, W, mode="exposed")
            st2["ps"].image.copy_(st["ps"].image)
            st2["ps"].labels.copy_(st["ps"].labels)
            farr, fn = st2["plan"].fwd_cmds
            barr, bn = st2["plan"].bwd_cmds
            self._run_cmds(farr, 0, fn, sp)
            self._run_cmds(barr, 0, bn, sp)
            cands = {"overlap": st, "exposed": st2}
            best = {}
            for mode, s_ in cands.items():
                self._ddp_build_env(mode)
                if self.use_graph and s_["graphs"] is None:
                    self._capture(s_)
            ev0, ev1 = torch.cuda.Event(enable_timing=True), torch.cuda.Event(enable_timing=True)
            for r in range(rounds):
                for mode, s_ in cands.items():
                    self._ddp_build_env(mode)
                    self.stream.synchronize()
                    dist.barrier()
                    ev0.record(self.stream)
                    for _ in range(reps):
                        self._run_backward(s_)
                    ev1.record(self.stream)
                    ev1.synchronize()
                    ms = ev0.elapsed_time(ev1) / reps
                    best[mode] = ms if mode not in best else min(best[mode], ms)
            t = torch.tensor([best["overlap"], best["exposed"]], device=self.params.data.device, dtype=torch.float64)
            dist.all_reduce(t, op=dist.ReduceOp.MAX)
            t_ov, t_ex = float(t[0]), float(t[1])
            for tns, v in saved:
                tns.copy_(v)
        mode = "overlap" if t_ov <= t_ex else "exposed"
        self.ddp_choice = dict(mode=mode, selected_on_device=dict(overlap_backward_ms=round(t_ov, 4), exposed_backward_ms=round(t_ex, 4)),
                               rule="max over ranks of the best of %d rounds x %d backward passes incl. all-reduce" % (rounds, reps))
        self.ddp_mode, self.ddp_auto = mode, False
        self._ddp_build_env(mode)
        for k in [k for k in self._states if len(k) == 4]:
            self._states.pop(k)
        if mode == "exposed":
            st2["warm"] = True
            keep = {k: st[k] for k in ("stage", "stage_k") if k in st}
            st.clear()
            st.update(st2)
            st.update(keep)
        self._states[(B, H, W)] = st

    def _run_cmds(self, arr, lo, hi, sp):
        if hi > lo:
            ptr = C.cast(C.byref(arr, lo * C.sizeof(L.mi_cmd)), C.POINTER(L.mi_cmd))
            L.check(L.lib().mi_cmdlist_run(ptr, hi - lo, sp), "cmdlist_run")

    def _capture(self, st):
        lib, s = L.lib(), self.stream
        sp = L.stream_ptr(s)
        plan = st["plan"]
        farr, fn = plan.fwd_cmds
        barr, bn = plan.bwd_cmds
        gs = {"fwd": L.check(lib.mi_graph_capture(farr, fn, sp), "capture fwd"), "bwd": [], "fwd_stage": {}}
        for (lo, hi, bucket) in st["segs"]:
            h = None
            if hi > lo:
                ptr = C.cast(C.byref(barr, lo * C.sizeof(L.mi_cmd)), C.POINTER(L.mi_cmd))
                h = L.check(lib.mi_graph_capture(ptr, hi - lo, sp), "capture bwd segment")
            gs["bwd"].append(h)
        gs["sgd"] = L.check(lib.mi_graph_capture(st["sgd"], 1, sp), "capture sgd")
        gs["step"], gs["step_stage"] = None, {}
        if self.one_graph and self.world == 1:
            arr, n = self._whole_step_cmds(st, farr, fn)
            gs["step"] = L.check(lib.mi_graph_capture(arr, n, sp), "capture whole step")
        st["graphs"] = gs

    def _whole_step_cmds(self, st, farr, fn):
        barr, bn = st["plan"].bwd_cmds
        sz = C.sizeof(L.mi_cmd)
        arr = (L.mi_cmd * (fn + bn + 1))()
        C.memmove(arr, farr, fn * sz)
        C.memmove(C.byref(arr, fn * sz), barr, bn * sz)
        C.memmove(C.byref(arr, (fn + bn) * sz), st["sgd"], sz)
        st.setdefault("_step_arrays", []).append(arr)
        return arr, fn + bn + 1

    def load_batch(self, images, labels):
        B, _, H, W = images.shape
        st = self._state(B, H, W)
        self.stream.wait_stream(torch.cuda.current_stream())
        with torch.cuda.stream(self.stream):
            st["ps"].image.copy_(images, non_blocking=True)
            st["ps"].labels.copy_(labels, non_blocking=True)
        for t in (images, labels):
            if t.is_cuda:
                t.record_stream(self.stream)
        return st

    def feed(self, st, images_host, labels_host):
        if self.copy_stream is None:
            self.copy_stream = torch.cuda.Stream()
        if "stage" not in st:
            ps = st["ps"]
            st["stage"] = []
            for k in range(2):
                lab_flat = torch.zeros_like(ps.labels_flat)
                st["stage"].append(dict(img=torch.empty_like(ps.image), lab_flat=lab_flat,
                                        lab=lab_flat[:ps.labels.numel()].view(ps.labels.shape), k=k,
                                        ready=torch.cuda.Event(), free=torch.cuda.Event(), st=st))
            st["stage_k"] = 0
            for b in st["stage"]:
                b["free"].record(self.stream)
        b = st["stage"][st["stage_k"]]
        st["stage_k"] ^= 1
        if tuple(images_host.shape) != tuple(b["img"].shape) or tuple(labels_host.shape) != tuple(b["lab"].shape):
            raise ValueError(f"feed(): batch {tuple(images_host.shape)} / {tuple(labels_host.shape)} does not match the "
                             f"state's input buffers {tuple(b['img'].shape)} / {tuple(b['lab'].shape)}")
        b["free"].synchronize()
        with torch.cuda.stream(self.copy_stream):
            b["img"].copy_(images_host, non_blocking=True)
            b["lab"].copy_(labels_host, non_blocking=True)
            b["ready"].record(self.copy_stream)
        self._feed = b

    def _staged_fwd(self, st, k):
        key = ("fwd_stage_cmds", k)
        if key in st:
            return st[key]
        ps, b = st["ps"], st["stage"][k]
        farr, fn = st["plan"].fwd_cmds
        arr = (L.mi_cmd * (fn + 1))()
        c = arr[0]
        c.op = L.OP["COPY"]
        c.p[0], c.p[1] = b["lab_flat"].data_ptr(), ps.labels_flat.data_ptr()
        c.i[0], c.i[1], c.i[2], c.i[3] = 8, 8, 0, 8
        c.l[0] = ps.labels_flat.numel() // 4
        C.memmove(C.byref(arr, C.sizeof(L.mi_cmd)), farr, fn * C.sizeof(L.mi_cmd))
        img = ps.image.data_ptr()
        hits = [j for j in range(1, fn + 1) if arr[j].op == L.OP["FOCUS"] and arr[j].p[0] == img]
        if len(hits) != 1:
            raise L.MI355Error(f"staged forward: expected one Focus command reading the plan's image, found {len(hits)}")
        arr[hits[0]].p[0] = b["img"].data_ptr()
        st[key] = (arr, fn + 1)
        return st[key]

    def step(self, st):
        lib = L.lib()
        plan, red = st["plan"], st["red"]
        with torch.cuda.stream(self.stream):
            sp = L.stream_ptr(self.stream)
            staged = None
            if self._feed is not None:
                b, self._feed = self._feed, None
                if b["st"] is not st:
                    raise ValueError("step(): the batch handed to feed() belongs to another input shape's state")
                self.stream.wait_event(b["ready"])
                if self.feed_direct:
                    staged = b
                else:
                    st["ps"].image.copy_(b["img"], non_blocking=True)
                    st["ps"].labels.copy_(b["lab"], non_blocking=True)
                    b["free"].record(self.stream)
            if self.ddp_auto and st.get("warm"):
                self._choose_ddp_schedule(st)
                plan, red = st["plan"], st["red"]
            if self.use_graph and st["graphs"] is None:
                if st.get("warm"):
                    if self.tune:
                        self.tune_report = plan.autotune_convs(stream=self.stream)
                    self._capture(st)
                st["warm"] = True
            gs = st["graphs"] if self.use_graph else None
            farr, fn = plan.fwd_cmds
            barr, bn = plan.bwd_cmds
            if gs and gs.get("step") is not None:
                if staged is not None:
                    h = gs["step_stage"].get(staged["k"])
                    if h is None:
                        sarr, sn = self._staged_fwd(st, staged["k"])
                        arr, n = self._whole_step_cmds(st, sarr, sn)
                        h = gs["step_stage"][staged["k"]] = L.check(lib.mi_graph_capture(arr, n, sp), "capture staged whole step")
                        gs["fwd_stage"][staged["k"]] = h
                    L.check(lib.mi_graph_launch(h, sp), "launch staged whole step")
                    staged["free"].record(self.stream)
                else:
                    L.check(lib.mi_graph_launch(gs["step"], sp), "launch whole step")
                return
            if staged is not None:
                sarr, sn = self._staged_fwd(st, staged["k"])
                if gs:
                    h = gs["fwd_stage"].get(staged["k"])
                    if h is None:
                        h = gs["fwd_stage"][staged["k"]] = L.check(lib.mi_graph_capture(sarr, sn, sp), "capture staged fwd")
                    L.check(lib.mi_graph_launch(h, sp), "launch staged fwd")
                else:
                    self._run_cmds(sarr, 0, sn, sp)
                staged["free"].record(self.stream)
            elif gs:
                L.check(lib.mi_graph_launch(gs["fwd"], sp), "launch fwd")
            else:
                self._run_cmds(farr, 0, fn, sp)
            for i, (lo, hi, bucket) in enumerate(st["segs"]):
                if gs:
                    if gs["bwd"][i] is not None:
                        L.check(lib.mi_graph_launch(gs["bwd"][i], sp), "launch bwd")
                else:
                    self._run_cmds(barr, lo, hi, sp)
                red.reduce_bucket(bucket)
            red.wait()
            if gs:
                L.check(lib.mi_graph_launch(gs["sgd"], sp), "launch sgd")
            else:
                self._run_cmds(st["sgd"], 0, 1, sp)

    def losses(self, st):
        self.stream.synchronize()
        st["plan"].check_bn_barriers()
        return st["ps"].loss_out().cpu()
```

yolov7_d2_amd/params.py:

```python
import torch

from . import _lib as L


class ParamArena:
    def __init__(self, module: torch.nn.Module, device):
        self.device = torch.device(device)
        self.entries = []
        off = 0
        named = list(module.named_parameters())
        order = [n for n, _ in named]
        for mname, m in module.named_modules():
            fn = getattr(m, "arena_adjacent", None)
            if fn is None:
                continue
            pre = mname + "." if mname else ""
            for a, b in fn():
                a, b = pre + a, pre + b
                if a in order and b in order:
                    order.remove(b)
                    order.insert(order.index(a) + 1, b)
        byname = dict(named)
        for name in order:
            p = byname[name]
            n = p.numel()
            self.entries.append((name, p, off, n))
            off += (n + 3) // 4 * 4
        self.total = off
        self.data = torch.zeros(off, dtype=torch.float32, device=self.device)
        self.grad = torch.zeros(off, dtype=torch.float32, device=self.device)
        self.mom = torch.zeros(off, dtype=torch.float32, device=self.device)
        self._grad_views = {}
        with torch.no_grad():
            for name, p, o, n in self.entries:
                v = self.data[o:o + n].view(p.shape)
                v.copy_(p.data.to(self.device, torch.float32))
                p.data = v
                self._grad_views[id(p)] = self.grad[o:o + n].view(p.shape)
        self._segs = None

    def grad_of(self, p):
        return self._grad_views[id(p)]

    def bind_grads(self):
        for name, p, o, n in self.entries:
            p.grad = self._grad_views[id(p)]

    def build_sgd_segments(self, lr, weight_decay, weight_decay_norm, norm_param_ids, chunk=16384):
        segs = []
        for name, p, o, n in self.entries:
            wd = weight_decay_norm if id(p) in norm_param_ids else weight_decay
            k = 0
            while k < n:
                c = min(chunk, n - k)
                segs.append((o + k, c, wd, lr))
                k += c
        arr = (L.mi_sgd_seg * len(segs))()
        for i, (o, c, wd, l_) in enumerate(segs):
            arr[i].offset, arr[i].count, arr[i].weight_decay, arr[i].lr = o, c, wd, l_
        host = torch.frombuffer(bytearray(bytes(arr)), dtype=torch.uint8).clone()
        self._segs_host = arr
        self._segs = host.to(self.device)
        self._nseg = len(segs)
        return self._segs, self._nseg

    def set_lr(self, lr):
        arr = self._segs_host
        for i in range(self._nseg):
            arr[i].lr = lr
        host = torch.frombuffer(bytearray(bytes(arr)), dtype=torch.uint8)
        self._segs.copy_(host, non_blocking=False)
```

yolov7_d2_amd/plan.py:

```python
import ctypes as C
import math
import os

import torch

from . import _lib as L


def _rup(a, b):
    return (a + b - 1) // b * b


class Buf:

    def __init__(self, name, nbytes, zero=False):
        self.name, self.nbytes, self.offset, self.zero = name, int(nbytes), None, zero
        self.base = None

    @property
    def ptr(self):
        return self.base + self.offset


class TRef:
# ... 649 lines not shown
        best = {}
        handles = {}
        keep = {}
        for fused in (True, False):
            self.bn_fused = fused
            self._materialize_bwd()
            arr, n = self.bwd_cmds
            keep[fused] = (self.bwd_cmds, self.bwd_tags, self.cmd_descs["bwd"], self.cmd_members["bwd"],
                           list(self.wgrad_descs), list(getattr(self, "wgrad_stage_tags", [])), self.cmd_objs["bwd"])
            with torch.cuda.stream(s):
                L.check(lib.mi_cmdlist_run(arr, n, sp), "bn select: eager run")
                handles[fused] = L.check(lib.mi_graph_capture(arr, n, sp), "bn select: capture")
        with torch.cuda.stream(s):
            for r in range(rounds + 1):
                for fused in (True, False):
                    a, e = torch.cuda.Event(enable_timing=True), torch.cuda.Event(enable_timing=True)
                    a.record(s)
                    for _ in range(launches):
                        L.check(lib.mi_graph_launch(handles[fused], sp), "bn select: launch")
                    e.record(s)
                    e.synchronize()
                    if r > 0:
                        t = a.elapsed_time(e) / launches
                        best[fused] = min(best.get(fused, 1e9), t)
        for h in handles.values():
            lib.mi_graph_destroy(h)
        self.bn_fused_timing = dict(fused_ms=round(best[True], 4), two_pass_ms=round(best[False], 4))
        self.bn_fused = best[True] <= best[False]
        (self.bwd_cmds, self.bwd_tags, self.cmd_descs["bwd"], self.cmd_members["bwd"], self.wgrad_descs,
         self.wgrad_stage_tags, self.cmd_objs["bwd"]) = keep[self.bn_fused]

    def _group_wgrads(self, bwd):
        b = self.b
        wg = [c for c in bwd if c.op == L.OP["WGRAD"]]
        self.wgrad_descs = []
        if not (b.group_wgrad and len(wg) >= 2):
            return bwd
        stages, rest = [], list(wg)
        if b.wgrad_split:
            for pre in b.wgrad_stages:
                st = [c for c in rest if c.tag.startswith(tuple(pre))]
                if len(st) >= 2:
                    stages.append(st)
                    rest = [c for c in rest if not any(c is x for x in st)]
        if len(rest) < 2:
            if stages:
                rest = stages.pop() + rest
        pos = {id(c): i for i, c in enumerate(bwd)}
        issue_at = {max(pos[id(c)] for c in st): si for si, st in enumerate(stages)}
        out = []
        for i, c in enumerate(bwd):
            if c.op != L.OP["WGRAD"]:
                out.append(c)
            if i in issue_at:
                si = issue_at[i]
                out.append(self._wgrad_group_cmd(stages[si], "wgrad_group.early" if si == 0 else f"wgrad_group.stage{si}"))
        out.append(self._wgrad_group_cmd(rest, "wgrad_group"))
        self.wgrad_stage_tags = [[c.tag for c in st] for st in stages] + [[c.tag for c in rest]]
        return out

    def _wgrad_group_cmd(self, wg, tag):
        ws = self.b.wgrad_group_ws
        descs = (L.mi_wgrad_desc * len(wg))()
        for d, c in zip(descs, wg):
            t = PlanBuilder._wgrad_desc(c.desc)
            t.x, t.dy, t.gw = c.desc.x.resolve(), c.desc.dy.resolve(), c.desc.gw.resolve()
            C.memmove(C.byref(d), C.byref(t), C.sizeof(L.mi_wgrad_desc))
        meta = L.mi_wgrad_group()
        L.check(L.lib().mi_conv2d_wgrad_group_plan(descs, len(wg), ws.ptr, None, 0, C.byref(meta)), "wgrad_group_plan")
        assert meta.ws_bytes <= ws.nbytes, (meta.ws_bytes, ws.nbytes)
        host = (C.c_char * int(meta.table_bytes))()
        L.check(L.lib().mi_conv2d_wgrad_group_plan(descs, len(wg), ws.ptr, host, meta.table_bytes, C.byref(meta)),
                "wgrad_group_plan")
        table = self._upload_table(host, meta.table_bytes)
        if meta.ngroups > 0 and meta.g[0].fixup:
            nbytes = min(int(meta.g[k].job_off) for k in range(meta.ngroups)) // 256 * 256
            if not hasattr(self, "wgrad_fix_tables"):
                self.wgrad_fix_tables = []
            self.wgrad_fix_tables.append((table, nbytes))
        self.descs += [meta, descs]
        self.wgrad_descs += list(descs)
        grp = _Cmd(L.OP["WGRAD_GROUP"], p=[_Ptr(C.addressof(meta)), _Ptr(table)], tag=tag)
        grp.group_descs = list(descs)
        grp.parts = list(wg)
        return grp

    def _fuse_bn_bwd_pairs(self, bwd):
        RED, APP = L.OP["BN_BWD_REDUCE"], L.OP["BN_BWD_APPLY"]
        out, k = [], 0
        while k < len(bwd):
            c = bwd[k]
            n = bwd[k + 1] if k + 1 < len(bwd) else None
            if (c.op == RED and n is not None and n.op == APP and c.tag.endswith(".bnred")
                    and n.tag == c.tag[:-len(".bnred")] + ".bnapply" and len(n.p) > 12 and n.p[12].obj is not None):
                f = _Cmd(L.OP["BN_BWD_FUSED"], i=n.i, l=n.l, p=n.p, tag=c.tag[:-len(".bnred")] + ".bnbwd")
                f.lane = n.lane
                f.members = [c, n]
                out.append(f)
                k += 2
            else:
                out.append(c)
                k += 1
        return out

    def _batch_splits(self, bwd):
        sp = [c for c in bwd if c.op == L.OP["SPLIT_DPREDS"]]
        if not (self.b.group_wgrad and 2 <= len(sp) <= 16) or os.environ.get("MI_SPLIT_BATCH", "1") == "0":
            return bwd
        at = max(k for k, c in enumerate(bwd) if c.op in (L.OP["LOSS_BWD"], L.OP["BIAS_GRADS"]))
        assert all(k > at for k, c in enumerate(bwd) if c.op == L.OP["SPLIT_DPREDS"])
        B, A, nch = sp[0].i[:3]
        spec = ConvSpec(kind="split_jobs", jobs=[dict(dst=c.p[1], a0=c.i[3], HW=c.i[4], c0=c.i[5], nc=c.i[6], ld=c.i[7])
                                                 for c in sp])
        cmd = _Cmd(L.OP["SPLIT_DPREDS_BATCH"], i=[B, A, nch, len(sp)], p=[_Ptr(None), sp[0].p[0]], desc=spec,
                   tag="loss.split_all")
        cmd.lane = bwd[at].lane
        cmd.members = list(sp)
        rest = [c for c in bwd if c.op != L.OP["SPLIT_DPREDS"]]
        k = next(k for k, c in enumerate(rest) if c is bwd[at])
        return rest[:k + 1] + [cmd] + rest[k + 1:]

    def _fuse_loss_bwd(self, bwd):
        if os.environ.get("MI_LOSS_BWD_FUSED", "1") == "0":
            return bwd
        ops = [c.op for c in bwd]
        try:
            k = ops.index(L.OP["LOSS_BWD"])
        except ValueError:
            return bwd
        if ops[k + 1: k + 3] != [L.OP["BIAS_GRADS"], L.OP["SPLIT_DPREDS_BATCH"]]:
            return bwd
        lb, bg, sp = bwd[k: k + 3]
        B, A, nch = sp.i[:3]
        cells = sum(j["HW"] * j["nc"] for j in sp.desc.jobs)
        if cells != A * nch or len(sp.desc.jobs) > 16:
            return bwd
        sj, bj = self._make_desc(sp.desc), self._make_desc(bg.desc)
        keep = os.environ.get("MI_LOSS_DPREDS", "0") == "1"
        cmd = _Cmd(L.OP["LOSS_BWD_FUSED"], i=[len(sp.desc.jobs), len(bg.desc.jobs)], l=[bg.p[2].obj.nbytes // 4], desc=lb.desc,
                   p=[_Ptr(None), lb.p[1], lb.p[2] if keep else _Ptr(None), _Ptr(C.addressof(sj)), _Ptr(C.addressof(bj)), bg.p[2]],
                   tag="loss.bwd_fused")
        cmd.lane = getattr(lb, "lane", 0)
        cmd.members = [lb, bg] + list(sp.members)
        cmd.bias_jobs = bj
        return bwd[:k] + [cmd] + bwd[k + 3:]

    def _batch_packs(self, prologue):
        packs = [c for c in prologue if c.op == L.OP["PACK_W"]]
        rest = [c for c in prologue if c.op != L.OP["PACK_W"]]
        if len(packs) < 2:
            return prologue
        jobs = (L.mi_pack_job * len(packs))()
        for j, c in zip(jobs, packs):
            Cout, Cin, KH, KW, CinPad, CoutPad, CoutPadK, CinPadN = c.i[:8]
            j.w, j.wf, j.wd = c.p[0].resolve(), c.p[1].resolve(), c.p[2].resolve()
            j.Cout, j.Cin, j.KK, j.CinPad, j.CoutPad, j.CoutPadK, j.CinPadN = Cout, Cin, KH * KW, CinPad, CoutPad, CoutPadK, CinPadN
        nblk = L.check(L.lib().mi_pack_jobs_layout(jobs, len(packs)), "pack_jobs_layout")
        tab = torch.frombuffer(bytearray(bytes(jobs)), dtype=torch.uint8).to(self.b.device)
        self.pack_table = tab
        cmd = _Cmd(L.OP["PACK_W_BATCH"], i=[len(packs), nblk, max(j.KK for j in jobs)], p=[_Ptr(tab)], tag="pack_all")
        cmd.parts = packs
        return rest + [cmd]

    def _make_desc(self, spec):
        kind = getattr(spec, "kind", "conv")
        if kind == "conv":
            d = L.mi_conv_desc()
            d.x, d.w, d.y = spec.x.resolve(), spec.w.resolve(), spec.y.resolve()
            d.bias, d.stats_acc = spec.bias.resolve(), spec.stats.resolve()
            for k in ("ldx", "ldy", "y_nstride", "N", "H", "W", "outH", "outW", "gridH", "gridW", "in_stride",
                      "out_stride", "out_oy", "out_ox", "K8", "Cout", "CoutPad", "flags", "stats_slots"):
                setattr(d, k, int(getattr(spec, k)))
            d.ntaps = len(spec.taps)
            for t, (dy, dx, w) in enumerate(spec.taps):
                d.tap_dy[t], d.tap_dx[t], d.tap_w[t] = dy, dx, w
            if getattr(spec, "tps", 0):
                d.TPS = int(spec.tps)
            xf = getattr(spec, "xf", None)
            if xf is not None:
                d.xf, d.xf_write, d.xf_C = xf.resolve(), int(spec.xf_write), int(spec.xf_C)
            bnb = getattr(spec, "bnb", None)
            if bnb is not None:
                d.bn_y, d.bn_ldy, d.bn_act = bnb["y"].resolve(), bnb["ldy"], bnb["act"]
                d.bn_scale, d.bn_shift = bnb["scale"].resolve(), bnb["shift"].resolve()
                d.bn_mean, d.bn_invstd = bnb["mean"].resolve(), bnb["invstd"].resolve()
        elif kind == "bias_jobs":
            d = (L.mi_bias_job * len(spec.jobs))()
            for jd, j in zip(d, spec.jobs):
                jd.out, jd.a0, jd.HW, jd.c0, jd.nc = j["out"].data_ptr(), j["a0"], j["HW"], j["c0"], j["nc"]
        elif kind == "split_jobs":
            d = (L.mi_split_job * len(spec.jobs))()
            for jd, j in zip(d, spec.jobs):
                jd.dst, jd.a0, jd.HW, jd.c0, jd.nc, jd.ld = j["dst"].resolve(), j["a0"], j["HW"], j["c0"], j["nc"], j["ld"]
        elif kind == "wgrad":
            d = PlanBuilder._wgrad_desc(spec)
            d.x, d.dy, d.gw = spec.x.resolve(), spec.dy.resolve(), spec.gw.resolve()
            d.ws, d.ws_bytes = spec.ws.ptr, spec.ws.nbytes
        else:
            d = L.mi_yolox_loss_desc()
            d.preds, d.labels, d.anchors = spec.preds.resolve(), spec.labels.resolve(), spec.anchors.resolve()
            d.B, d.A, d.ncls, d.max_labels, d.gmax = spec.B, spec.A, spec.ncls, spec.max_labels, spec.gmax
            for k in ("cost", "iou", "match", "ngt", "fg", "matched_gt", "matched_iou", "partial", "out", "partial_l1"):
                setattr(d, k, spec.ws[k].ptr)
            d.use_l1 = int(getattr(spec, "use_l1", False))
        self.descs.append(d)
        return d

    def _group_lanes(self, cmds):
        NOP, CONV = L.OP["NOP"], L.OP["CONV"]
        BN_KIND = {L.OP["BN_ACT_FWD"]: 0, L.OP["BN_BWD_REDUCE"]: 1, L.OP["BN_BWD_APPLY"]: 2, L.OP["BN_BWD_FUSED"]: 3}

        def issue(cs, order):
            cs = sorted(cs, key=lambda c: order[id(c)])
            if len(cs) < 2:
                return cs
            if cs[0].op == CONV:
                parts = [cs]
                if os.environ.get("MI_GROUP_LONG", "1") == "0":
                    def nblocks(c):
                        d = self._make_desc(c.desc)
                        self.descs.pop()
                        n_ = L.lib().mi_conv2d_plan(C.byref(d))
                        return max(n_, 1) * (d.CoutPad // d.BN), (d.K8 * 8 // d.KC) * (d.ntaps // d.TPS)
                    info = [nblocks(c) for c in cs]
                    if not all(st <= 2 for _, st in info):
                        parts, cur, tot = [], [], 0
                        for c, (nb_, _) in sorted(zip(cs, info), key=lambda t: t[1][0]):
                            if nb_ >= 384 or tot + nb_ > 640:
                                if cur:
                                    parts.append(cur)
                                cur, tot = [], 0
                            if nb_ >= 384:
                                parts.append([c])
                            else:
                                cur.append(c)
                                tot += nb_
                        if cur:
                            parts.append(cur)
                res = []
                for part in parts:
                    part = sorted(part, key=lambda c: order[id(c)])
                    g = self._conv_group_cmd(part) if len(part) >= 2 else None
# ... 519 lines not shown
```

Measured before the change: 3065 images/sec.

## Fuse wgrad split-reduce, SGD update and weight repack into one step-tail kernel

```diff
diff --git a/include/mi355_det.h b/include/mi355_det.h
--- a/include/mi355_det.h
+++ b/include/mi355_det.h
@@ -129,6 +129,9 @@
 int mi_conv2d_wgrad_group_plan(const mi_wgrad_desc* descs, int n, void* ws_base, void* table_host,
                                int64_t table_cap, mi_wgrad_group* meta);
 int mi_conv2d_wgrad_group_run(const mi_wgrad_group* meta, const void* table_dev, mi_stream_t s);
+#define MI_WGRAD_PART_GRIDS 1
+#define MI_WGRAD_PART_REDUCE 2
+int mi_conv2d_wgrad_group_run_parts(const mi_wgrad_group* meta, const void* table_dev, int parts, mi_stream_t s);
 int mi_upload_async(void* dst_dev, const void* src_pinned, int64_t nbytes, mi_stream_t s);
 
 int mi_pack_conv_weight(const float* w_oihw, int Cout, int Cin, int KH, int KW,
@@ -456,6 +459,33 @@
                          int first_step, mi_stream_t s);
 
 int mi_sigmoid_f32(const float* x, const float* dy, float* y, float* dx, int64_t n, mi_stream_t s);
+typedef struct mi_tail_job {
+  int32_t kind;
+  int32_t blk0, nblk;
+  int32_t seg0, nseg;
+  int32_t chunk;
+  int32_t Cout, Cin, KK, CinPad, CoutPad, CoutPadK, CinPadN;
+  int32_t nco_t;
+  int32_t nsplit, MI, NJ, WCO, WCI, nco, nci, bld;
+  int64_t off;
+  int64_t V;
+  const float* part;
+  const float* row_scale;
+  const float* scale;
+  void* wf;
+  void* wd;
+} mi_tail_job;
+typedef struct mi_step_tail {
+  int32_t njobs, nblocks, lds_bytes, keep_grad;
+  int32_t ntile_jobs, nbias_jobs, nflat_jobs, pad_;
+  int64_t table_bytes;
+} mi_step_tail;
+int mi_step_tail_plan(const mi_wgrad_desc* descs, int n, void* ws_base, const mi_pack_job* packs, int npacks,
+                      const mi_sgd_seg* segs_host, int nseg, const float* params, const float* grads, int keep_grad,
+                      void* table_host, int64_t table_cap, mi_step_tail* meta);
+int mi_step_tail_run(const mi_step_tail* meta, const void* table_dev, float* params, float* grads, float* momentum_buf,
+                     const mi_sgd_seg* segs_dev, float momentum, float grad_scale, int first_step, mi_stream_t s);
+
 int mi_adamw_step(float* params, const float* grads, float* exp_avg, float* exp_avg_sq, const mi_sgd_seg* segs_dev,
                   int nseg, float beta1, float beta2, float eps, int64_t step, float grad_scale, mi_stream_t s);
 typedef struct mi_adamw_tensor {
@@ -578,6 +608,7 @@
   MI_OP_DWCONV_DGRAD = 35,
   MI_OP_DWCONV_WGRAD = 36,
   MI_OP_LOSS_BWD_FUSED = 37,
+  MI_OP_STEP_TAIL = 38,
   MI_OP_COUNT
 };
 
diff --git a/yolov7_d2_amd/_lib.py b/yolov7_d2_amd/_lib.py
--- a/yolov7_d2_amd/_lib.py
+++ b/yolov7_d2_amd/_lib.py
@@ -150,6 +150,21 @@
                 ("scale", C.c_void_p)]
 
 
+class mi_tail_job(C.Structure):
+    _fields_ = ([(n, C.c_int32) for n in ("kind", "blk0", "nblk", "seg0", "nseg", "chunk", "Cout", "Cin", "KK", "CinPad", "CoutPad",
+                                         "CoutPadK", "CinPadN", "nco_t", "nsplit", "MI", "NJ", "WCO", "WCI", "nco", "nci", "bld")] +
+                [("off", C.c_int64), ("V", C.c_int64)] +
+                [(n, C.c_void_p) for n in ("part", "row_scale", "scale", "wf", "wd")])
+
+
+class mi_step_tail(C.Structure):
+    _fields_ = [(n, C.c_int32) for n in ("njobs", "nblocks", "lds_bytes", "keep_grad", "ntile_jobs", "nbias_jobs", "nflat_jobs",
+                                         "pad_")] + [("table_bytes", C.c_int64)]
+
+
+WGRAD_PART_GRIDS, WGRAD_PART_REDUCE = 1, 2
+
+
 class mi_sparseinst_loss_desc(C.Structure):
     _fields_ = [(n, C.c_void_p) for n in ("logits", "scores", "labels", "match_q", "match_t", "nmatch", "inv_num", "stats", "gup",
                                           "pairs", "valid", "row_cls", "row_pair", "kdev", "losses", "dlogits", "dscores", "coef")] + \
@@ -225,7 +240,7 @@
        "RESERVED8", "BN_BWD_APPLY", "FOCUS", "UPSAMPLE_FWD", "UPSAMPLE_BWD", "SPP_FWD", "SPP_BWD", "COPY",
        "COLSUM", "LOSS_FWD", "LOSS_BWD", "SPLIT_DPREDS", "MEMSET", "SGD", "BN_EVAL_AFFINE", "DECODE", "PACK_W_BATCH", "WGRAD_GROUP", "RESERVED26", "RESERVED27", "RESERVED28", "BIAS_GRADS",
        "CONV_GROUP", "BN_GROUP", "SPLIT_DPREDS_BATCH", "BN_BWD_FUSED", "DWCONV_FWD", "DWCONV_DGRAD", "DWCONV_WGRAD",
-       "LOSS_BWD_FUSED"]
+       "LOSS_BWD_FUSED", "STEP_TAIL"]
 OP = {n: k for k, n in enumerate(OPS)}
 
 _vp, _i, _i64, _f = C.c_void_p, C.c_int, C.c_int64, C.c_float
@@ -238,6 +253,10 @@
     "mi_conv2d_wgrad": (C.c_int, [C.POINTER(mi_wgrad_desc), _vp]),
     "mi_conv2d_wgrad_group_plan": (C.c_int, [C.POINTER(mi_wgrad_desc), _i, _vp, _vp, _i64, C.POINTER(mi_wgrad_group)]),
     "mi_conv2d_wgrad_group_run": (C.c_int, [C.POINTER(mi_wgrad_group), _vp, _vp]),
+    "mi_conv2d_wgrad_group_run_parts": (C.c_int, [C.POINTER(mi_wgrad_group), _vp, _i, _vp]),
+    "mi_step_tail_plan": (C.c_int, [C.POINTER(mi_wgrad_desc), _i, _vp, C.POINTER(mi_pack_job), _i, C.POINTER(mi_sgd_seg), _i,
+                                    _vp, _vp, _i, _vp, _i64, C.POINTER(mi_step_tail)]),
+    "mi_step_tail_run": (C.c_int, [C.POINTER(mi_step_tail), _vp, _vp, _vp, _vp, _vp, _f, _f, _i, _vp]),
     "mi_pack_conv_weight": (C.c_int, [_vp, _i, _i, _i, _i, _vp, _i, _i, _vp, _i, _i, _vp]),
     "mi_pack_conv_weight_scaled": (C.c_int, [_vp, _vp, _i, _i, _i, _i, _vp, _i, _i, _vp, _i, _i, _vp]),
     "mi_scale_rows_f32": (C.c_int, [_vp, _vp, _vp, _i, _i, _vp]),
diff --git a/yolov7_d2_amd/csrc/conv_wgrad.hip b/yolov7_d2_amd/csrc/conv_wgrad.hip
--- a/yolov7_d2_amd/csrc/conv_wgrad.hip
+++ b/yolov7_d2_amd/csrc/conv_wgrad.hip
@@ -2,6 +2,7 @@
 #include <string.h>
 #include <vector>
 #include "common.h"
+#include "wgrad_reduce.h"
 
 struct Wg2K {
   const __bf16* x;
@@ -687,16 +688,6 @@
   wgrad3_body<NT, MI, NJ, WCO, WCI, TP, true>(p, b - starts[j], (unsigned*)((char*)const_cast<Wg2K*>(jobs) + p.cnt_rel));
 }
 
-struct Wg2R {
-  const f32x4* part;
-  float* g;
-  long long V;
-  int nsplit, NT, MI, NJ, WCO, WCI, nco, nci, Cout, Cin, accumulate;
-  const float* row_scale;
-  const float* bpart;
-  float* gbias;
-  int bld, main_blocks;
-};
 __device__ __forceinline__ void wgrad2_reduce_bias(const Wg2R& p, const long long blk) {
   const int c = (int)(blk - p.main_blocks) * 256 + (int)threadIdx.x;
   if (c >= p.Cout) return;
@@ -1305,10 +1296,17 @@
 }
 
 extern "C" int mi_conv2d_wgrad_group_run(const mi_wgrad_group* meta, const void* table_dev, mi_stream_t st) {
+  return mi_conv2d_wgrad_group_run_parts(meta, table_dev, MI_WGRAD_PART_GRIDS | MI_WGRAD_PART_REDUCE, st);
+}
+
+extern "C" int mi_conv2d_wgrad_group_run_parts(const mi_wgrad_group* meta, const void* table_dev, int parts, mi_stream_t st) {
   MI_REQUIRE(meta && table_dev && meta->ngroups > 0, "wgrad_group_run: args");
+  MI_REQUIRE(parts & (MI_WGRAD_PART_GRIDS | MI_WGRAD_PART_REDUCE), "wgrad_group_run: parts %d", parts);
+  MI_REQUIRE(parts == (MI_WGRAD_PART_GRIDS | MI_WGRAD_PART_REDUCE) || !meta->g[0].fixup,
+             "wgrad_group_run: a group that sums its own partials (MI_WG_FIXUP=1) has no separate reduce part");
   hipStream_t s = (hipStream_t)st;
   const char* tab = (const char*)table_dev;
-  for (int gi = 0; gi < meta->ngroups; ++gi) {
+  for (int gi = 0; gi < meta->ngroups && (parts & MI_WGRAD_PART_GRIDS); ++gi) {
     const auto& g = meta->g[gi];
     const Wg2K* jobs = (const Wg2K*)(tab + g.job_off);
     const int* starts = (const int*)(tab + g.starts_off);
@@ -1350,6 +1348,7 @@
     if (rc == MI_EINVAL) MI_FAIL(MI_EINVAL, "wgrad_group: no kernel for group %d", gi);
     if (rc) return rc;
   }
+  if (!(parts & MI_WGRAD_PART_REDUCE)) return MI_OK;
   if (meta->red9_blocks > 0) {
     hipLaunchKernelGGL(wgrad2_reduce9_group_kernel, dim3((unsigned)meta->red9_blocks), dim3(576), 0, s,
                        (const Wg2R*)(tab + meta->red9_off), (const int*)(tab + meta->red9_starts_off), meta->nred9);
diff --git a/yolov7_d2_amd/csrc/misc_ops.hip b/yolov7_d2_amd/csrc/misc_ops.hip
--- a/yolov7_d2_amd/csrc/misc_ops.hip
+++ b/yolov7_d2_amd/csrc/misc_ops.hip
@@ -1,5 +1,6 @@
 #include <stdlib.h>
 #include "common.h"
+#include "sgd_update.h"
 
 static int ew_blocks(int64_t total, int cap = 4096) {
   int64_t b = (total + 255) / 256;
@@ -866,40 +867,7 @@
 __global__ __launch_bounds__(256) void sgd_kernel(float* p, const float* __restrict__ g, float* m,
                                                   const mi_sgd_seg* __restrict__ segs, float momentum,
                                                   float grad_scale, int first_step) {
-  const mi_sgd_seg sg = segs[blockIdx.x];
-  const float wd = sg.weight_decay, lr = sg.lr;
-  const int64_t n4 = ((sg.offset & 3) == 0) ? (sg.count >> 2) : 0;
-  f32x4* p4 = (f32x4*)(p + sg.offset);
-  const f32x4* g4 = (const f32x4*)(g + sg.offset);
-  f32x4* m4 = (f32x4*)(m + sg.offset);
-  for (int64_t i = threadIdx.x; i < n4; i += 512) {
-    const bool two = i + 256 < n4;
-    const f32x4 pa = p4[i], ga = g4[i], ma = first_step ? f32x4{0.f, 0.f, 0.f, 0.f} : m4[i];
-    f32x4 pb = {0.f, 0.f, 0.f, 0.f}, gb = pb, mb = pb;
-    if (two) {
-      pb = p4[i + 256];
-      gb = g4[i + 256];
-      if (!first_step) mb = m4[i + 256];
-    }
-    f32x4 da = ga * grad_scale + pa * wd;
-    f32x4 ba = first_step ? da : ma * momentum + da;
-    m4[i] = ba;
-    p4[i] = pa - ba * lr;
-    if (two) {
-      f32x4 db = gb * grad_scale + pb * wd;
-      f32x4 bb = first_step ? db : mb * momentum + db;
-      m4[i + 256] = bb;
-      p4[i + 256] = pb - bb * lr;
-    }
-  }
-  for (int64_t i = n4 * 4 + threadIdx.x; i < sg.count; i += 256) {
-    const int64_t k = sg.offset + i;
-    const float pv = p[k];
-    const float d = g[k] * grad_scale + wd * pv;
-    const float b = first_step ? d : momentum * m[k] + d;
-    m[k] = b;
-    p[k] = pv - lr * b;
-  }
+  sgd_seg_body(p, g, m, segs[blockIdx.x], momentum, grad_scale, first_step);
 }
 extern "C" int mi_sgd_momentum_step(float* params, const float* grads, float* momentum_buf,
                                     const mi_sgd_seg* segs_dev, int nseg, float momentum, float grad_scale,
diff --git a/yolov7_d2_amd/csrc/runtime.hip b/yolov7_d2_amd/csrc/runtime.hip
--- a/yolov7_d2_amd/csrc/runtime.hip
+++ b/yolov7_d2_amd/csrc/runtime.hip
@@ -69,7 +69,12 @@
     case MI_OP_COLSUM: return mi_colsum_bf16(p[0], i[0], c.l[0], i[1], (float*)p[1], i[2], (float*)p[2], st);
     case MI_OP_BIAS_GRADS:
       return mi_yolox_bias_grads((const float*)p[1], i[0], i[1], i[2], (const mi_bias_job*)p[0], i[3], (float*)p[2], st);
-    case MI_OP_WGRAD_GROUP: return mi_conv2d_wgrad_group_run((const mi_wgrad_group*)p[0], p[1], st);
+    case MI_OP_WGRAD_GROUP:
+      return mi_conv2d_wgrad_group_run_parts((const mi_wgrad_group*)p[0], p[1],
+                                             i[0] ? i[0] : (MI_WGRAD_PART_GRIDS | MI_WGRAD_PART_REDUCE), st);
+    case MI_OP_STEP_TAIL:
+      return mi_step_tail_run((const mi_step_tail*)p[0], p[1], (float*)p[2], (float*)p[3], (float*)p[4],
+                              (const mi_sgd_seg*)p[5], c.f[0], c.f[1], i[0], st);
     case MI_OP_CONV_GROUP: return mi_conv2d_group_run((const mi_conv_group*)p[0], p[1], st);
     case MI_OP_BN_GROUP: return mi_bn_group_run((const mi_bn_group*)p[0], p[1], st);
     case MI_OP_PACK_W_BATCH: return mi_pack_conv_weights_batch((const mi_pack_job*)p[0], i[0], i[1], i[2], st);
diff --git a/yolov7_d2_amd/csrc/sgd_update.h b/yolov7_d2_amd/csrc/sgd_update.h
--- /dev/null
+++ b/yolov7_d2_amd/csrc/sgd_update.h
@@ -0,0 +1,56 @@
+#pragma once
+#include "common.h"
+
+__device__ __forceinline__ void sgd_seg_body(float* p, const float* __restrict__ g, float* m, const mi_sgd_seg sg,
+                                             const float momentum, const float grad_scale, const int first_step) {
+  const float wd = sg.weight_decay, lr = sg.lr;
+  const int64_t n4 = ((sg.offset & 3) == 0) ? (sg.count >> 2) : 0;
+  f32x4* p4 = (f32x4*)(p + sg.offset);
+  const f32x4* g4 = (const f32x4*)(g + sg.offset);
+  f32x4* m4 = (f32x4*)(m + sg.offset);
+  for (int64_t i = threadIdx.x; i < n4; i += 512) {
+    const bool two = i + 256 < n4;
+    const f32x4 pa = p4[i], ga = g4[i], ma = first_step ? f32x4{0.f, 0.f, 0.f, 0.f} : m4[i];
+    f32x4 pb = {0.f, 0.f, 0.f, 0.f}, gb = pb, mb = pb;
+    if (two) {
+      pb = p4[i + 256];
+      gb = g4[i + 256];
+      if (!first_step) mb = m4[i + 256];
+    }
+    f32x4 da = ga * grad_scale + pa * wd;
+    f32x4 ba = first_step ? da : ma * momentum + da;
+    m4[i] = ba;
+    p4[i] = pa - ba * lr;
+    if (two) {
+      f32x4 db = gb * grad_scale + pb * wd;
+      f32x4 bb = first_step ? db : mb * momentum + db;
+      m4[i + 256] = bb;
+      p4[i + 256] = pb - bb * lr;
+    }
+  }
+  for (int64_t i = n4 * 4 + threadIdx.x; i < sg.count; i += 256) {
+    const int64_t k = sg.offset + i;
+    const float pv = p[k];
+    const float d = g[k] * grad_scale + wd * pv;
+    const float b = first_step ? d : momentum * m[k] + d;
+    m[k] = b;
+    p[k] = pv - lr * b;
+  }
+}
+
+__device__ __forceinline__ void sgd_upd4(f32x4& p, f32x4& m, const f32x4 ga, const float wd, const float lr,
+                                         const float momentum, const float grad_scale, const int first_step) {
+  const f32x4 pa = p, ma = first_step ? f32x4{0.f, 0.f, 0.f, 0.f} : m;
+  f32x4 da = ga * grad_scale + pa * wd;
+  f32x4 ba = first_step ? da : ma * momentum + da;
+  m = ba;
+  p = pa - ba * lr;
+}
+__device__ __forceinline__ void sgd_upd1(float& p, float& m, const float gv, const float wd, const float lr,
+                                         const float momentum, const float grad_scale, const int first_step) {
+  const float pv = p;
+  const float d = gv * grad_scale + wd * pv;
+  const float b = first_step ? d : momentum * m + d;
+  m = b;
+  p = pv - lr * b;
+}
diff --git a/yolov7_d2_amd/csrc/step_tail.hip b/yolov7_d2_amd/csrc/step_tail.hip
--- /dev/null
+++ b/yolov7_d2_amd/csrc/step_tail.hip
@@ -0,0 +1,432 @@
+#include <algorithm>
+#include <string.h>
+#include <vector>
+#include "common.h"
+#include "sgd_update.h"
+#include "wgrad_reduce.h"
+
+#define TL_CO 16
+#define TL_CI 64
+#define TL_U 3
+
+struct TailArgs {
+  const mi_tail_job* jobs;
+  float* p;
+  float* g;
+  float* m;
+  const mi_sgd_seg* segs;
+  float momentum, grad_scale;
+  int njobs, first_step, keep_grad, rs;
+};
+
+__device__ __forceinline__ int tl_seg_of(const mi_tail_job& j, const mi_sgd_seg* __restrict__ segs, const long long e) {
+  if (j.nseg == 1) return j.seg0;
+  if (j.chunk > 0) return j.seg0 + (int)((unsigned)(e - j.off) / (unsigned)j.chunk);
+  int lo = j.seg0, hi = j.seg0 + j.nseg - 1;
+  while (lo < hi) {
+    const int mid = (lo + hi + 1) >> 1;
+    if (segs[mid].offset <= e) lo = mid; else hi = mid - 1;
+  }
+  return lo;
+}
+
+__device__ __forceinline__ long long tl_frag_v(const mi_tail_job& j, const int cf, const int cif, const int tap) {
+  const int mw = j.MI * j.WCO, nw = j.NJ * j.WCI;
+  const int cob = cf / mw, r = cf - cob * mw, wco = r / j.MI, i = r - wco * j.MI;
+  const int cib = cif / nw, r2 = cif - cib * nw, wci = r2 / j.NJ, jj = r2 - wci * j.NJ;
+  const long long wave = wco * j.WCI + wci;
+  return ((((((long long)cob * j.nci + cib) * (j.WCO * j.WCI) + wave) * j.KK + tap) * j.MI + i) * j.NJ + jj) * 64;
+}
+
+__device__ __forceinline__ f32x4 tl_sum_long(const f32x4* __restrict__ src, const long long V, const int nsplit) {
+  const f32x4 z = {0.f, 0.f, 0.f, 0.f};
+  f32x4 tot = z;
+#pragma unroll
+  for (int h = 0; h < 2; ++h) {
+    f32x4 s[2][4];
+#pragma unroll
+    for (int q = 0; q < 2; ++q)
+#pragma unroll
+      for (int e = 0; e < 4; ++e) s[q][e] = z;
+    int k0 = 2 * h, k1 = 2 * h + 1;
+    for (; k1 + 12 < nsplit; k0 += 16, k1 += 16) {
+      f32x4 a[2][4];
+#pragma unroll
+      for (int e = 0; e < 4; ++e) {
+        a[0][e] = src[(size_t)(k0 + 4 * e) * V];
+        a[1][e] = src[(size_t)(k1 + 4 * e) * V];
+      }
+#pragma unroll
+      for (int e = 0; e < 4; ++e) { s[0][e] += a[0][e]; s[1][e] += a[1][e]; }
+    }
+    if (k0 + 12 < nsplit) {
+      f32x4 a[4];
+#pragma unroll
+      for (int e = 0; e < 4; ++e) a[e] = src[(size_t)(k0 + 4 * e) * V];
+#pragma unroll
+      for (int e = 0; e < 4; ++e) s[0][e] += a[e];
+      k0 += 16;
+    }
+    for (; k0 < nsplit || k1 < nsplit; k0 += 4, k1 += 4) {
+      f32x4 a = z, b = z;
+      if (k0 < nsplit) a = src[(size_t)k0 * V];
+      if (k1 < nsplit) b = src[(size_t)k1 * V];
+      if (k0 < nsplit) s[0][0] += a;
+      if (k1 < nsplit) s[1][0] += b;
+    }
+    const f32x4 u0 = (s[0][0] + s[0][1]) + (s[0][2] + s[0][3]);
+    const f32x4 u1 = (s[1][0] + s[1][1]) + (s[1][2] + s[1][3]);
+    if (h == 0) tot = u0; else tot += u0;
+    tot += u1;
+  }
+  return tot;
+}
+
+__device__ __forceinline__ unsigned tl_bf16_word(const float v) {
+  return (unsigned)__builtin_bit_cast(unsigned short, (__bf16)v);
+}
+
+__device__ __forceinline__ void tl_tile(const TailArgs& a, const mi_tail_job& j, const int t, float* const tl_s) {
+  const int tid = threadIdx.x, wave = tid >> 6, lane = tid & 63;
+  const int KK = j.KK, rs = a.rs;
+  const int co0 = (t % j.nco_t) * TL_CO, ci0 = (t / j.nco_t) * TL_CI;
+  int nci = j.Cin - ci0;
+  nci = nci < 0 ? 0 : (nci > TL_CI ? TL_CI : nci);
+  const int rowlen = TL_CI * KK, nval = nci * KK;
+  const long long e00 = j.off + ((long long)co0 * j.Cin + ci0) * KK;
+  const long long rowstep = (long long)j.Cin * KK;
+
+  if (j.part) {
+    const int nfrag = 4 * KK;
+    const int cf = co0 >> 4;
+    const bool cf_ok = cf < j.nco * j.MI * j.WCO;
+    const int ncif = j.nci * j.NJ * j.WCI;
+    const int nsplit = j.nsplit;
+    const long long V = j.V;
+    const f32x4* const part = (const f32x4*)j.part;
+    const int r4 = 4 * (lane >> 4), c16 = lane & 15;
+    for (int f0 = wave; f0 < nfrag; f0 += 4 * TL_U) {
+      f32x4 tot[TL_U];
+      bool ok[TL_U];
+      const f32x4* src[TL_U];
+#pragma unroll
+      for (int u = 0; u < TL_U; ++u) {
+        const int f = f0 + 4 * u;
+        const int cif = (ci0 >> 4) + (f & 3);
+        ok[u] = f < nfrag && cf_ok && cif < ncif;
+        src[u] = part + (ok[u] ? tl_frag_v(j, cf, cif, f >> 2) : 0) + lane;
+        tot[u] = f32x4{0.f, 0.f, 0.f, 0.f};
+      }
+      if (nsplit <= 12) {
+        f32x4 s[TL_U][4];
+#pragma unroll
+        for (int u = 0; u < TL_U; ++u)
+#pragma unroll
+          for (int sl = 0; sl < 4; ++sl) s[u][sl] = f32x4{0.f, 0.f, 0.f, 0.f};
+        for (int k = 0; k < nsplit; k += 4) {
+          f32x4 ld[TL_U][4];
+#pragma unroll
+          for (int u = 0; u < TL_U; ++u)
+#pragma unroll
+            for (int sl = 0; sl < 4; ++sl) {
+              ld[u][sl] = f32x4{0.f, 0.f, 0.f, 0.f};
+              if (ok[u] && k + sl < nsplit) ld[u][sl] = src[u][(size_t)(k + sl) * V];
+            }
+#pragma unroll
+          for (int u = 0; u < TL_U; ++u)
+#pragma unroll
+            for (int sl = 0; sl < 4; ++sl)
+              if (k + sl < nsplit) s[u][sl] += ld[u][sl];
+        }
+#pragma unroll
+        for (int u = 0; u < TL_U; ++u) tot[u] = ((s[u][0] + s[u][1]) + s[u][2]) + s[u][3];
+      } else {
+#pragma unroll
+        for (int u = 0; u < TL_U; ++u)
+          if (ok[u]) tot[u] = tl_sum_long(src[u], V, nsplit);
+      }
+#pragma unroll
+      for (int u = 0; u < TL_U; ++u) {
+        const int f = f0 + 4 * u;
+        if (f >= nfrag) continue;
+        float* dst = tl_s + r4 * rs + ((f & 3) * 16 + c16) * KK + (f >> 2);
+#pragma unroll
+        for (int e = 0; e < 4; ++e) {
+          const int co = co0 + r4 + e;
+          float v = tot[u][e];
+          if (j.row_scale && co < j.Cout) v = __fmul_rn(v, j.row_scale[co]);
+          dst[e * rs] = v;
+        }
+      }
+    }
+  } else {
+    for (int idx = tid; idx < TL_CO * rowlen; idx += 256) {
+      const int co_l = idx / rowlen, q = idx - co_l * rowlen;
+      float v = 0.f;
+      if (co0 + co_l < j.Cout && q < nval) v = a.g[e00 + co_l * rowstep + q];
+      tl_s[co_l * rs + q] = v;
+    }
+  }
+  __syncthreads();
+
+  unsigned* const tl_w = (unsigned*)tl_s;
+  const bool vec = (rowstep & 3) == 0 && (nval & 3) == 0 && (j.off & 3) == 0 && (j.nseg == 1 || (j.chunk > 0 && (j.chunk & 3) == 0));
+  if (vec) {
+    const int r4n = rowlen >> 2;
+    for (int idx = tid; idx < TL_CO * r4n; idx += 256) {
+      const int co_l = idx / r4n, q = (idx - co_l * r4n) * 4;
+      const int co = co0 + co_l;
+      u32x4 w = {0u, 0u, 0u, 0u};
+      if (co < j.Cout && q < nval) {
+        const long long e = e00 + co_l * rowstep + q;
+        const mi_sgd_seg sg = a.segs[tl_seg_of(j, a.segs, e)];
+        const f32x4 gv = *(const f32x4*)(tl_s + co_l * rs + q);
+        f32x4 pv = *(const f32x4*)(a.p + e);
+        f32x4 mv = {0.f, 0.f, 0.f, 0.f};
+        if (!a.first_step) mv = *(const f32x4*)(a.m + e);
+        sgd_upd4(pv, mv, gv, sg.weight_decay, sg.lr, a.momentum, a.grad_scale, a.first_step);
+        *(f32x4*)(a.m + e) = mv;
+        *(f32x4*)(a.p + e) = pv;
+        if (a.keep_grad) *(f32x4*)(a.g + e) = gv;
+        const float sc = j.scale ? j.scale[co] : 1.f;
+        w = u32x4{tl_bf16_word(pv[0] * sc), tl_bf16_word(pv[1] * sc), tl_bf16_word(pv[2] * sc), tl_bf16_word(pv[3] * sc)};
+      }
+      *(u32x4*)(tl_w + co_l * rs + q) = w;
+    }
+  } else {
+    for (int idx = tid; idx < TL_CO * rowlen; idx += 256) {
+      const int co_l = idx / rowlen, q = idx - co_l * rowlen;
+      const int co = co0 + co_l;
+      unsigned w = 0u;
+      if (co < j.Cout && q < nval) {
+        const long long e = e00 + co_l * rowstep + q;
+        const mi_sgd_seg sg = a.segs[tl_seg_of(j, a.segs, e)];
+        const float gv = tl_s[co_l * rs + q];
+        float pv = a.p[e];
+        float mv = a.first_step ? 0.f : a.m[e];
+        sgd_upd1(pv, mv, gv, sg.weight_decay, sg.lr, a.momentum, a.grad_scale, a.first_step);
+        a.m[e] = mv;
+        a.p[e] = pv;
+        if (a.keep_grad) a.g[e] = gv;
+        float v = pv;
+        if (j.scale) v *= j.scale[co];
+        w = tl_bf16_word(v);
+      }
+      tl_w[co_l * rs + q] = w;
+    }
+  }
+  __syncthreads();
+
+  const unsigned short* const hs = (const unsigned short*)tl_s;
+  const int K8f = j.CinPad / 8, K8d = j.CoutPadK / 8;
+  if (j.wf) {
+    for (int it = tid; it < KK * 128; it += 256) {
+      const int tap = it >> 7, k8_l = (it >> 4) & 7, co_l = it & 15;
+      const int k8 = ci0 / 8 + k8_l, co = co0 + co_l;
+      if (k8 >= K8f || co >= j.CoutPad) continue;
+      unsigned h[8];
+#pragma unroll
+      for (int e = 0; e < 8; ++e) h[e] = hs[2 * (co_l * rs + (k8_l * 8 + e) * KK + tap)];
+      ((uint4*)j.wf)[((size_t)tap * K8f + k8) * j.CoutPad + co] =
+          make_uint4(h[0] | (h[1] << 16), h[2] | (h[3] << 16), h[4] | (h[5] << 16), h[6] | (h[7] << 16));
+    }
+  }
+  if (j.wd) {
+    for (int it = tid; it < KK * 128; it += 256) {
+      const int tap = it >> 7, co8_l = (it >> 6) & 1, ci_l = it & 63;
+      const int co8 = co0 / 8 + co8_l, ci = ci0 + ci_l;
+      if (co8 >= K8d || ci >= j.CinPadN) continue;
+      unsigned h[8];
+#pragma unroll
+      for (int e = 0; e < 8; ++e) h[e] = hs[2 * ((co8_l * 8 + e) * rs + ci_l * KK + tap)];
+      ((uint4*)j.wd)[((size_t)tap * K8d + co8) * j.CinPadN + ci] =
+          make_uint4(h[0] | (h[1] << 16), h[2] | (h[3] << 16), h[4] | (h[5] << 16), h[6] | (h[7] << 16));
+    }
+  }
+}
+
+__global__ __launch_bounds__(256) void step_tail_kernel(const TailArgs a) {
+  extern __shared__ __attribute__((aligned(16))) float tl_s[];
+  const int b = blockIdx.x;
+  int lo = 0, hi = a.njobs - 1;
+  while (lo < hi) {
+    const int mid = (lo + hi + 1) >> 1;
+    if (a.jobs[mid].blk0 <= b) lo = mid; else hi = mid - 1;
+  }
+  const mi_tail_job j = a.jobs[lo];
+  const int t = b - j.blk0;
+  if (j.kind == 2) {
+    sgd_seg_body(a.p, a.g, a.m, a.segs[j.seg0 + t], a.momentum, a.grad_scale, a.first_step);
+    return;
+  }
+  if (j.kind == 1) {
+    const int c = t * 256 + (int)threadIdx.x;
+    if (c >= j.Cout) return;
+    float s = 0.f;
+    for (int k = 0; k < j.nsplit; ++k) s += j.part[(size_t)k * j.bld + c];
+    const long long e = j.off + c;
+    const mi_sgd_seg sg = a.segs[tl_seg_of(j, a.segs, e)];
+    float pv = a.p[e];
+    float mv = a.first_step ? 0.f : a.m[e];
+    sgd_upd1(pv, mv, s, sg.weight_decay, sg.lr, a.momentum, a.grad_scale, a.first_step);
+    a.m[e] = mv;
+    a.p[e] = pv;
+    if (a.keep_grad) a.g[e] = s;
+    return;
+  }
+  tl_tile(a, j, t, tl_s);
+}
+
+static int tl_rs(int kk_max) { return TL_CI * kk_max + 4; }
+
+extern "C" int mi_step_tail_plan(const mi_wgrad_desc* descs, int n, void* ws_base, const mi_pack_job* packs, int npacks,
+                                 const mi_sgd_seg* segs, int nseg, const float* params, const float* grads, int keep_grad,
+                                 void* table_host, int64_t table_cap, mi_step_tail* meta) {
+  MI_REQUIRE(n >= 0 && (n == 0 || descs) && npacks >= 0 && (npacks == 0 || packs) && segs && nseg > 0 && params && grads && meta,
+             "step_tail_plan: args");
+  memset(meta, 0, sizeof(*meta));
+  for (int s = 1; s < nseg; ++s)
+    MI_REQUIRE(segs[s].offset >= segs[s - 1].offset + segs[s - 1].count && segs[s - 1].count > 0,
+               "step_tail_plan: segment %d overlaps its predecessor or is out of order", s);
+  std::vector<Wg2R> red;
+  if (n > 0) {
+    mi_wgrad_group wm;
+    int rc = mi_conv2d_wgrad_group_plan(descs, n, ws_base, nullptr, 0, &wm);
+    if (rc) return rc;
+    std::vector<char> tab((size_t)wm.table_bytes);
+    rc = mi_conv2d_wgrad_group_plan(descs, n, ws_base, tab.data(), wm.table_bytes, &wm);
+    if (rc) return rc;
+    MI_REQUIRE(wm.nred9 == 0 && wm.nred == n && !wm.g[0].fixup,
+               "step_tail_plan: the group has no plain reduce job per layer (MI_WG_FIXUP / MI_WG_RED9 set?)");
+    red.resize((size_t)n);
+    memcpy(red.data(), tab.data() + wm.red_off, (size_t)n * sizeof(Wg2R));
+  }
+  auto seg_range = [&](int64_t lo, int64_t hi, int* s0, int* ns) -> bool {
+    int a = 0;
+    while (a < nseg && segs[a].offset < lo) ++a;
+    int b = a;
+    int64_t at = lo;
+    while (b < nseg && segs[b].offset == at && segs[b].offset + segs[b].count <= hi) { at += segs[b].count; ++b; }
+    *s0 = a; *ns = b - a;
+    return at == hi && b > a;
+  };
+  std::vector<char> seg_used((size_t)nseg, 0);
+  std::vector<char> red_used((size_t)n, 0);
+  std::vector<mi_tail_job> tiles, biases, flats;
+  int kk_max = 1;
+  for (int k = 0; k < npacks; ++k) {
+    const mi_pack_job& pj = packs[k];
+    MI_REQUIRE(pj.w && (pj.wf || pj.wd) && pj.KK >= 1 && pj.KK <= MI_MAX_TAPS, "step_tail_plan: pack job %d: null / taps", k);
+    if (pj.wf) MI_REQUIRE(pj.CinPad % 8 == 0 && pj.CinPad >= pj.Cin && pj.CoutPad >= pj.Cout, "step_tail_plan: pack job %d: fwd pads", k);
+    if (pj.wd) MI_REQUIRE(pj.CoutPadK % 8 == 0 && pj.CoutPadK >= pj.Cout && pj.CinPadN >= pj.Cin, "step_tail_plan: pack job %d: dgrad pads", k);
+    mi_tail_job j;
+    memset(&j, 0, sizeof(j));
+    j.kind = 0;
+    j.off = (int64_t)(pj.w - params);
+    const int64_t cnt = (int64_t)pj.Cout * pj.Cin * pj.KK;
+    MI_REQUIRE(pj.w >= params && cnt < (1LL << 31), "step_tail_plan: pack job %d: its weight lies outside the arena", k);
+    MI_REQUIRE(seg_range(j.off, j.off + cnt, &j.seg0, &j.nseg), "step_tail_plan: pack job %d: no run of segments covers exactly its weight", k);
+    for (int s = j.seg0; s < j.seg0 + j.nseg; ++s) {
+      MI_REQUIRE(!seg_used[s], "step_tail_plan: pack job %d shares segment %d with another job", k, s);
+      seg_used[s] = 1;
+    }
+    j.chunk = 0;
+    if (j.nseg > 1) {
+      bool uni = true;
+      for (int s = j.seg0; s + 1 < j.seg0 + j.nseg; ++s) uni = uni && segs[s].count == segs[j.seg0].count;
+      uni = uni && segs[j.seg0 + j.nseg - 1].count <= segs[j.seg0].count && segs[j.seg0].count < (1LL << 30);
+      if (uni) j.chunk = (int32_t)segs[j.seg0].count;
+    }
+    j.Cout = pj.Cout; j.Cin = pj.Cin; j.KK = pj.KK; j.CinPad = pj.CinPad; j.CoutPad = pj.CoutPad;
+    j.CoutPadK = pj.CoutPadK; j.CinPadN = pj.CinPadN; j.scale = pj.scale; j.wf = pj.wf; j.wd = pj.wd;
+    const int coP = pj.wd && pj.CoutPadK > pj.CoutPad ? pj.CoutPadK : (pj.wf ? pj.CoutPad : pj.CoutPadK);
+    const int ciP = pj.wd && pj.CinPadN > pj.CinPad ? pj.CinPadN : (pj.wf ? pj.CinPad : pj.CinPadN);
+    j.nco_t = (coP + TL_CO - 1) / TL_CO;
+    j.nblk = j.nco_t * ((ciP + TL_CI - 1) / TL_CI);
+    if (pj.KK > kk_max) kk_max = pj.KK;
+    for (int r = 0; r < n; ++r)
+      if (red[r].g - grads == j.off) {
+        const Wg2R& w = red[r];
+        MI_REQUIRE(!red_used[r], "step_tail_plan: two pack jobs share the weight of wgrad job %d", r);
+        MI_REQUIRE(w.Cout == pj.Cout && w.Cin == pj.Cin && w.NT == pj.KK && !w.accumulate,
+                   "step_tail_plan: wgrad job %d ([%d][%d][%d], accumulate %d) does not match pack job %d ([%d][%d][%d])", r,
+                   w.Cout, w.Cin, w.NT, w.accumulate, k, pj.Cout, pj.Cin, pj.KK);
+        red_used[r] = 1;
+        j.part = (const float*)w.part; j.V = w.V; j.nsplit = w.nsplit; j.MI = w.MI; j.NJ = w.NJ; j.WCO = w.WCO;
+        j.WCI = w.WCI; j.nco = w.nco; j.nci = w.nci; j.row_scale = w.row_scale;
+        MI_REQUIRE(w.nsplit >= 1 && (int64_t)w.nco * w.MI * w.WCO * 16 >= pj.Cout && (int64_t)w.nci * w.NJ * w.WCI * 16 >= pj.Cin,
+                   "step_tail_plan: wgrad job %d: its slabs do not cover the weight", r);
+        MI_REQUIRE(w.V == (int64_t)w.nco * w.nci * w.WCO * w.WCI * w.NT * w.MI * w.NJ * 64, "step_tail_plan: wgrad job %d: slab size", r);
+        if (w.bpart) {
+          mi_tail_job bj;
+          memset(&bj, 0, sizeof(bj));
+          bj.kind = 1;
+          bj.off = (int64_t)(w.gbias - grads);
+          bj.Cout = w.Cout; bj.nsplit = w.nsplit; bj.bld = w.bld; bj.part = w.bpart;
+          MI_REQUIRE(w.gbias >= grads && w.bld >= w.Cout, "step_tail_plan: wgrad job %d: bias gradient outside the arena", r);
+          MI_REQUIRE(seg_range(bj.off, bj.off + w.Cout, &bj.seg0, &bj.nseg), "step_tail_plan: wgrad job %d: no run of segments covers exactly its bias", r);
+          for (int s = bj.seg0; s < bj.seg0 + bj.nseg; ++s) {
+            MI_REQUIRE(!seg_used[s], "step_tail_plan: the bias of wgrad job %d shares segment %d with another job", r, s);
+            seg_used[s] = 1;
+          }
+          bj.nblk = (w.Cout + 255) / 256;
+          biases.push_back(bj);
+        }
+        break;
+      }
+    tiles.push_back(j);
+  }
+  for (int r = 0; r < n; ++r)
+    MI_REQUIRE(red_used[r], "step_tail_plan: wgrad job %d writes a weight that no pack job covers", r);
+  std::stable_sort(tiles.begin(), tiles.end(), [](const mi_tail_job& x, const mi_tail_job& y) {
+    return (int64_t)(x.part ? x.nsplit + 2 : 3) * x.KK > (int64_t)(y.part ? y.nsplit + 2 : 3) * y.KK;
+  });
+  for (int s = 0; s < nseg;) {
+    if (seg_used[s]) { ++s; continue; }
+    int e = s;
+    while (e < nseg && !seg_used[e]) ++e;
+    mi_tail_job j;
+    memset(&j, 0, sizeof(j));
+    j.kind = 2; j.seg0 = s; j.nseg = e - s; j.nblk = e - s; j.off = segs[s].offset;
+    flats.push_back(j);
+    s = e;
+  }
+  std::vector<mi_tail_job> all;
+  all.insert(all.end(), tiles.begin(), tiles.end());
+  all.insert(all.end(), biases.begin(), biases.end());
+  all.insert(all.end(), flats.begin(), flats.end());
+  int64_t blk = 0;
+  for (auto& j : all) {
+    j.blk0 = (int32_t)blk;
+    blk += j.nblk;
+    MI_REQUIRE(blk < (1LL << 30), "step_tail_plan: too many blocks");
+  }
+  meta->njobs = (int32_t)all.size(); meta->nblocks = (int32_t)blk; meta->keep_grad = keep_grad ? 1 : 0;
+  meta->ntile_jobs = (int32_t)tiles.size(); meta->nbias_jobs = (int32_t)biases.size(); meta->nflat_jobs = (int32_t)flats.size();
+  meta->lds_bytes = TL_CO * tl_rs(kk_max) * 4;
+  meta->table_bytes = (int64_t)(all.size() * sizeof(mi_tail_job));
+  if (table_host) {
+    MI_REQUIRE(meta->table_bytes <= table_cap, "step_tail_plan: table needs %lld bytes", (long long)meta->table_bytes);
+    memcpy(table_host, all.data(), (size_t)meta->table_bytes);
+  }
+  return MI_OK;
+}
+
+extern "C" int mi_step_tail_run(const mi_step_tail* meta, const void* table_dev, float* params, float* grads, float* momentum_buf,
+                                const mi_sgd_seg* segs_dev, float momentum, float grad_scale, int first_step, mi_stream_t st) {
+  MI_REQUIRE(meta && table_dev && params && grads && momentum_buf && segs_dev && meta->njobs > 0 && meta->nblocks > 0, "step_tail_run: args");
+  MI_REQUIRE(meta->lds_bytes >= TL_CO * tl_rs(1) * 4 && meta->lds_bytes <= TL_CO * tl_rs(MI_MAX_TAPS) * 4 && meta->lds_bytes % (TL_CO * 16) == 0,
+             "step_tail_run: lds_bytes %d", meta->lds_bytes);
+  static bool attr_done = false;
+  if (meta->lds_bytes > 64 * 1024 && !attr_done) {
+    hipFuncSetAttribute((const void*)step_tail_kernel, hipFuncAttributeMaxDynamicSharedMemorySize, 80 * 1024);
+    attr_done = true;
+  }
+  TailArgs a;
+  a.jobs = (const mi_tail_job*)table_dev; a.p = params; a.g = grads; a.m = momentum_buf; a.segs = segs_dev;
+  a.momentum = momentum; a.grad_scale = grad_scale; a.njobs = meta->njobs; a.first_step = first_step;
+  a.keep_grad = meta->keep_grad; a.rs = meta->lds_bytes / (TL_CO * 4);
+  hipLaunchKernelGGL(step_tail_kernel, dim3((unsigned)meta->nblocks), dim3(256), (size_t)meta->lds_bytes, (hipStream_t)st, a);
+  MI_CHECK_LAUNCH("step_tail");
+  return MI_OK;
+}
diff --git a/yolov7_d2_amd/csrc/wgrad_reduce.h b/yolov7_d2_amd/csrc/wgrad_reduce.h
--- /dev/null
+++ b/yolov7_d2_amd/csrc/wgrad_reduce.h
@@ -0,0 +1,13 @@
+#pragma once
+#include "common.h"
+
+struct Wg2R {
+  const f32x4* part;
+  float* g;
+  long long V;
+  int nsplit, NT, MI, NJ, WCO, WCI, nco, nci, Cout, Cin, accumulate;
+  const float* row_scale;
+  const float* bpart;
+  float* gbias;
+  int bld, main_blocks;
+};
diff --git a/yolov7_d2_amd/engine.py b/yolov7_d2_amd/engine.py
--- a/yolov7_d2_amd/engine.py
+++ b/yolov7_d2_amd/engine.py
@@ -26,8 +26,11 @@
 
 class NativeTrainer:
     def __init__(self, model, lr=0.01, momentum=0.9, weight_decay=1e-4, weight_decay_norm=0.0, n_buckets=3,
-                 use_graph=True, loss_weights=(1.0, 1.0, 1.0, 1.0), tune=None, input_u8=False):
+                 use_graph=True, loss_weights=(1.0, 1.0, 1.0, 1.0), tune=None, input_u8=False, keep_grad=False):
         self.model = model
+        self.step_tail = os.environ.get("MI_STEP_TAIL", "1") != "0"
+        self.keep_grad = bool(keep_grad)
+        self._packed = None
         self.input_u8 = bool(input_u8)
         self.copy_stream = None
         self._feed = None
@@ -187,13 +190,58 @@
             gs["step"] = L.check(lib.mi_graph_capture(arr, n, sp), "capture whole step")
         st["graphs"] = gs
 
+    def _tail(self, st):
+        if "tail" in st:
+            return st["tail"]
+        st["tail"] = None
+        plan = st["plan"]
+        farr, fn = plan.fwd_cmds
+        packs = [k for k in range(fn) if farr[k].op == L.OP["PACK_W_BATCH"]]
+        if not (self.step_tail and self.world == 1 and self.one_graph and self.use_graph and len(packs) == 1):
+            return None
+        t = plan.step_tail(self.params, keep_grad=self.keep_grad)
+        if t is None:
+            return None
+        barr, bn = plan.bwd_cmds
+        cmd = (L.mi_cmd * 1)()
+        cmd[0].op = L.OP["STEP_TAIL"]
+        cmd[0].p[0], cmd[0].p[1] = C.addressof(t["meta"]), t["table"].data_ptr()
+        cmd[0].p[2], cmd[0].p[3], cmd[0].p[4], cmd[0].p[5] = (self.params.data.data_ptr(), self.params._grad.data_ptr(),
+                                                              self.params.mom.data_ptr(), self.segs.data_ptr())
+        cmd[0].f[0], cmd[0].f[1] = self.momentum, 1.0
+        cmd[0].i[0] = 0
+        pack = (L.mi_cmd * 1)()
+        C.memmove(pack, C.byref(farr, packs[0] * C.sizeof(L.mi_cmd)), C.sizeof(L.mi_cmd))
+        red = (L.mi_cmd * 1)()
+        C.memmove(red, C.byref(barr, t["group"] * C.sizeof(L.mi_cmd)), C.sizeof(L.mi_cmd))
+        red[0].i[0] = L.WGRAD_PART_REDUCE
+        t.update(cmd=cmd, pack=pack, reduce=red, pack_at=packs[0])
+        st["tail"] = t
+        return t
+
+    def invalidate_packed(self):
+        self._packed = None
+
+    def _grad_from_partials(self, st):
+        with torch.cuda.stream(self.stream):
+            self._run_cmds(st["tail"]["reduce"], 0, 1, L.stream_ptr(self.stream))
+        torch.cuda.current_stream().wait_stream(self.stream)
+
     def _whole_step_cmds(self, st, farr, fn):
         barr, bn = st["plan"].bwd_cmds
         sz = C.sizeof(L.mi_cmd)
         arr = (L.mi_cmd * (fn + bn + 1))()
         C.memmove(arr, farr, fn * sz)
         C.memmove(C.byref(arr, fn * sz), barr, bn * sz)
-        C.memmove(C.byref(arr, (fn + bn) * sz), st["sgd"], sz)
+        tail = self._tail(st)
+        if tail is None:
+            C.memmove(C.byref(arr, (fn + bn) * sz), st["sgd"], sz)
+        else:
+            packs = [k for k in range(fn) if arr[k].op == L.OP["PACK_W_BATCH"]]
+            assert len(packs) == 1 and arr[fn + tail["group"]].op == L.OP["WGRAD_GROUP"]
+            arr[packs[0]].op = L.OP["NOP"]
+            arr[fn + tail["group"]].i[0] = L.WGRAD_PART_GRIDS
+            C.memmove(C.byref(arr, (fn + bn) * sz), tail["cmd"], sz)
         st.setdefault("_step_arrays", []).append(arr)
         return arr, fn + bn + 1
 
@@ -286,6 +334,14 @@
             farr, fn = plan.fwd_cmds
             barr, bn = plan.bwd_cmds
             if gs and gs.get("step") is not None:
+                tail = self._tail(st)
+                if tail is not None:
+                    ver = self.params.data._version
+                    if self._packed is None or self._packed[0] is not st or self._packed[1] != ver:
+                        self._run_cmds(tail["pack"], 0, 1, sp)
+                    self._packed = (st, ver)
+                    if not self.keep_grad:
+                        self.params.grad_pending = lambda st=st: self._grad_from_partials(st)
                 if staged is not None:
                     h = gs["step_stage"].get(staged["k"])
                     if h is None:
@@ -298,6 +354,7 @@
                 else:
                     L.check(lib.mi_graph_launch(gs["step"], sp), "launch whole step")
                 return
+            self._packed, self.params.grad_pending = None, None
             if staged is not None:
                 sarr, sn = self._staged_fwd(st, staged["k"])
                 if gs:
diff --git a/yolov7_d2_amd/params.py b/yolov7_d2_amd/params.py
--- a/yolov7_d2_amd/params.py
+++ b/yolov7_d2_amd/params.py
@@ -28,7 +28,8 @@
             off += (n + 3) // 4 * 4
         self.total = off
         self.data = torch.zeros(off, dtype=torch.float32, device=self.device)
-        self.grad = torch.zeros(off, dtype=torch.float32, device=self.device)
+        self.grad_pending = None
+        self._grad = torch.zeros(off, dtype=torch.float32, device=self.device)
         self.mom = torch.zeros(off, dtype=torch.float32, device=self.device)
         self._grad_views = {}
         with torch.no_grad():
@@ -39,7 +40,15 @@
                 self._grad_views[id(p)] = self.grad[o:o + n].view(p.shape)
         self._segs = None
 
+    @property
+    def grad(self):
+        if self.grad_pending is not None:
+            fn, self.grad_pending = self.grad_pending, None
+            fn()
+        return self._grad
+
     def grad_of(self, p):
+        self.grad
         return self._grad_views[id(p)]
 
     def bind_grads(self):
diff --git a/yolov7_d2_amd/plan.py b/yolov7_d2_amd/plan.py
--- a/yolov7_d2_amd/plan.py
+++ b/yolov7_d2_amd/plan.py
@@ -755,8 +755,31 @@
         self.wgrad_descs += list(descs)
         grp = _Cmd(L.OP["WGRAD_GROUP"], p=[_Ptr(C.addressof(meta)), _Ptr(table)], tag=tag)
         grp.group_descs = list(descs)
+        grp.group_desc_array = descs
         grp.parts = list(wg)
         return grp
+
+    def step_tail(self, params, keep_grad=False, host_only=False):
+        objs = self.cmd_objs["bwd"]
+        grp = [k for k, c in enumerate(objs) if c.op == L.OP["WGRAD_GROUP"]]
+        jobs = getattr(self, "pack_jobs", None)
+        if jobs is None or len(grp) != 1 or grp[0] != len(objs) - 1 or any(c.op == L.OP["WGRAD"] for c in objs):
+            return None
+        if (os.environ.get("MI_WG_FIXUP", "0") != "0" or os.environ.get("MI_WG_RED9", "0") != "0"
+                or os.environ.get("MI_WG_REDSL", "4") != "4"):
+            return None
+        descs = objs[grp[0]].group_desc_array
+        if any(d.accumulate for d in descs):
+            return None
+        segs = params._segs_host
+        meta = L.mi_step_tail()
+        args = (descs, len(descs), self.b.wgrad_group_ws.ptr, jobs, len(jobs), segs, len(segs), params.data.data_ptr(),
+                params.grad.data_ptr(), int(bool(keep_grad)))
+        L.check(L.lib().mi_step_tail_plan(*args, None, 0, C.byref(meta)), "step_tail_plan (sizes)")
+        host = (L.mi_tail_job * meta.njobs)()
+        L.check(L.lib().mi_step_tail_plan(*args, C.cast(host, C.c_void_p), C.sizeof(host), C.byref(meta)), "step_tail_plan")
+        table = host if host_only else self._upload_table(host, C.sizeof(host))
+        return dict(meta=meta, table=table, group=grp[0])
 
     def _fuse_bn_bwd_pairs(self, bwd):
         RED, APP = L.OP["BN_BWD_REDUCE"], L.OP["BN_BWD_APPLY"]
@@ -831,6 +854,7 @@
         nblk = L.check(L.lib().mi_pack_jobs_layout(jobs, len(packs)), "pack_jobs_layout")
         tab = torch.frombuffer(bytearray(bytes(jobs)), dtype=torch.uint8).to(self.b.device)
         self.pack_table = tab
+        self.pack_jobs = jobs
         cmd = _Cmd(L.OP["PACK_W_BATCH"], i=[len(packs), nblk, max(j.KK for j in jobs)], p=[_Ptr(tab)], tag="pack_all")
         cmd.parts = packs
         return rest + [cmd]
```

Result: slower. 2963 images/sec (-3.3%).
